# sai-soum/Diff-MST

Hardware: AMD Instinct MI355X
Metric: mixes/sec (8-track x 262144-sample fwd+bwd) (higher is better)
Workload: dtype f32

## Files before the change

### diff-mst_amd/csrc/mst_common.h

```cpp
#pragma once
#include <hip/hip_runtime.h>
#include <stdint.h>

#include "../../include/diffmst_hip.h"

namespace mst {

constexpr int kSections = 6;
constexpr int kStates = 2 * kSections;
#ifndef MST_COMP_WG
#define MST_COMP_WG 256
#endif
constexpr int kWG = MST_COMP_WG;
constexpr int kCompWaves = kWG / 64;
constexpr int kEqWG = 64;
constexpr int kEqChunk = 64;
constexpr int kCompChunk = 8;
constexpr int kScanThreads = 512;
constexpr int kScanLevels = 9;
constexpr int kPow = 1 + kScanLevels;
constexpr int kTile = kEqWG * kEqChunk;
constexpr int kPow1 = 12;
constexpr int kTri2 = 2 * 592;
constexpr int kFxDhChunks = 4;
constexpr int kWz = kEqChunk * 16;
constexpr int kMaxTiles1 = 64;

constexpr int RC_SOS = 0;
constexpr int RC_THR = 30;
constexpr int RC_KAPPA = 31;
constexpr int RC_KNEE = 32;
constexpr int RC_ALPHA = 33;
constexpr int RC_MAKEUP = 34;
constexpr int RC_ALPHA_C = 35;
constexpr int RC_PANL = 36;
constexpr int RC_PANR = 37;
constexpr int RC_GIN = 38;
constexpr int RC_LOG2A_C = 39;
constexpr int RC_SEND = 40;
constexpr int RC_AP = 44;
constexpr int RC_STRIDE = 64;

constexpr int CP_THR = 0, CP_KAPPA = 1, CP_KNEE = 2, CP_ALPHA = 3, CP_MAKEUP = 4, CP_PANL = 5, CP_PANR = 6, CP_SEND = 7;
constexpr int CP_COUNT = 8;
constexpr int EP_COUNT = 30;

constexpr float kDbPerLog2 = 6.02059991327962390f;
constexpr float kLog2PerDb = 0.16609640474436813f;
constexpr float kLn10Over20 = 0.11512925464970229f;
constexpr float kCompEps = 1e-8f;

__host__ __device__ inline int64_t round_up(int64_t a, int64_t b) { return (a + b - 1) / b * b; }
__host__ __device__ inline int filter_row(int sig, int split) { return sig < split ? sig : split + ((sig - split) >> 1); }

#if defined(__clang__)
using f2 = float __attribute__((ext_vector_type(2)));
__host__ __device__ __forceinline__ f2 f2_fma(f2 a, f2 b, f2 c) { return __builtin_elementwise_fma(a, b, c); }
#else
struct f2 {
    float x, y;
};
inline f2 operator*(f2 a, f2 b) { return f2{a.x * b.x, a.y * b.y}; }
inline f2 operator+(f2 a, f2 b) { return f2{a.x + b.x, a.y + b.y}; }
inline f2 f2_fma(f2 a, f2 b, f2 c) { return f2{fmaf(a.x, b.x, c.x), fmaf(a.y, b.y, c.y)}; }
#endif

template <typename T>
__device__ __forceinline__ T biquad_step(T x, const T* c, T& s1, T& s2) {
    T y = c[0] * x + s1;
    T n1 = c[1] * x + s2;
    s1 = n1 - c[3] * y;
    s2 = c[2] * x - c[4] * y;
    return y;
}
template <>
__device__ __forceinline__ float biquad_step<float>(float x, const float* c, float& s1, float& s2) {
    float y = fmaf(c[0], x, s1);
    float n1 = fmaf(c[1], x, s2);
    s1 = fmaf(-c[3], y, n1);
    s2 = fmaf(-c[4], y, c[2] * x);
    return y;
}

template <typename T>
__device__ __forceinline__ T cascade_step(T x, const T* c, T* st) {
#pragma unroll
    for (int k = 0; k < kSections; ++k) x = biquad_step<T>(x, c + 5 * k, st[2 * k], st[2 * k + 1]);
    return x;
}

template <typename T>
__device__ __forceinline__ T biquad_adj_step(T g, const T* c, T& r1, T& r2) {
    T p = g - c[3] * r1 - c[4] * r2;
    T xb = c[0] * p + c[1] * r1 + c[2] * r2;
    r2 = r1;
    r1 = p;
    return xb;
}
template <typename T>
__device__ __forceinline__ T cascade_adj_step(T g, const T* c, T* st) {
#pragma unroll
    for (int j = 0; j < kSections; ++j) {
        const int k = kSections - 1 - j;
        g = biquad_adj_step<T>(g, c + 5 * k, st[2 * j], st[2 * j + 1]);
    }
    return g;
}

__device__ __forceinline__ float4 load4(const float* __restrict__ row, int64_t i, int64_t n) {
    if (i + 3 < n && !((uintptr_t)(row + i) & 15)) return *reinterpret_cast<const float4*>(row + i);
    float4 v = make_float4(0.f, 0.f, 0.f, 0.f);
    if (i < n) v.x = row[i];
    if (i + 1 < n) v.y = row[i + 1];
    if (i + 2 < n) v.z = row[i + 2];
    if (i + 3 < n) v.w = row[i + 3];
    return v;
}
__device__ __forceinline__ void store4(float* __restrict__ row, int64_t i, int64_t n, float4 v) {
    if (i + 3 < n && !((uintptr_t)(row + i) & 15)) {
        *reinterpret_cast<float4*>(row + i) = v;
        return;
    }
    if (i < n) row[i] = v.x;
    if (i + 1 < n) row[i + 1] = v.y;
    if (i + 2 < n) row[i + 2] = v.z;
    if (i + 3 < n) row[i + 3] = v.w;
}
__device__ __forceinline__ float4 load4_shift(const float* __restrict__ row, int64_t i, int64_t n) {
    if (i >= 0 && i + 3 < n && !((uintptr_t)(row + i) & 15)) return *reinterpret_cast<const float4*>(row + i);
    float4 v = make_float4(0.f, 0.f, 0.f, 0.f);
    if (i >= 0 && i < n) v.x = row[i];
    if (i + 1 >= 0 && i + 1 < n) v.y = row[i + 1];
    if (i + 2 >= 0 && i + 2 < n) v.z = row[i + 2];
    if (i + 3 >= 0 && i + 3 < n) v.w = row[i + 3];
    return v;
}

__device__ __forceinline__ void wave_lds_sync() {
    __builtin_amdgcn_fence(__ATOMIC_RELEASE, "wavefront");
    __builtin_amdgcn_wave_barrier();
    __builtin_amdgcn_fence(__ATOMIC_ACQUIRE, "wavefront");
}

__device__ __forceinline__ void lds_barrier() {
    __builtin_amdgcn_fence(__ATOMIC_RELEASE, "workgroup", "local");
    __builtin_amdgcn_s_barrier();
    __builtin_amdgcn_fence(__ATOMIC_ACQUIRE, "workgroup", "local");
}
template <int LANES>
__device__ __forceinline__ void group_lds_sync() {
    if (LANES <= 64) wave_lds_sync();
    else lds_barrier();
}

template <int CTRL, int ROW_MASK>
__device__ __forceinline__ float dpp_add(float v) {
    return v + __int_as_float(__builtin_amdgcn_update_dpp(0, __float_as_int(v), CTRL, ROW_MASK, 0xf, true));
}
__device__ __forceinline__ float wave_sum(float v) {
    v = dpp_add<0x111, 0xf>(v);
    v = dpp_add<0x112, 0xf>(v);
    v = dpp_add<0x114, 0xf>(v);
    v = dpp_add<0x118, 0xf>(v);
    v = dpp_add<0x142, 0xa>(v);
    v = dpp_add<0x143, 0xc>(v);
    return __int_as_float(__builtin_amdgcn_readlane(__float_as_int(v), 63));
}

template <int CTRL, int ROW_MASK>
__device__ __forceinline__ double dpp_add_f64(double v) {
    const long long b = __double_as_longlong(v);
    const int lo = __builtin_amdgcn_update_dpp(0, (int)(b & 0xffffffffll), CTRL, ROW_MASK, 0xf, true);
    const int hi = __builtin_amdgcn_update_dpp(0, (int)(b >> 32), CTRL, ROW_MASK, 0xf, true);
    return v + __longlong_as_double(((long long)hi << 32) | (long long)(unsigned)lo);
}
__device__ __forceinline__ double wave_sum_f64(double v) {
    v = dpp_add_f64<0x111, 0xf>(v);
    v = dpp_add_f64<0x112, 0xf>(v);
    v = dpp_add_f64<0x114, 0xf>(v);
    v = dpp_add_f64<0x118, 0xf>(v);
    v = dpp_add_f64<0x142, 0xa>(v);
    v = dpp_add_f64<0x143, 0xc>(v);
    const long long b = __double_as_longlong(v);
    const int lo = __builtin_amdgcn_readlane((int)(b & 0xffffffffll), 63), hi = __builtin_amdgcn_readlane((int)(b >> 32), 63);
    return __longlong_as_double(((long long)hi << 32) | (long long)(unsigned)lo);
}

typedef unsigned long long gran_t;
#ifndef MST_GRAN_SPINS
#define MST_GRAN_SPINS (1 << 22)
#endif
constexpr int kStatusExchangeTimeout = 2000;
__device__ __forceinline__ void gran_give_up(int32_t* status) {
    if (status) atomicMax(status, kStatusExchangeTimeout);
}
__device__ __forceinline__ gran_t gran_load(const gran_t* g) { return __hip_atomic_load(g, __ATOMIC_RELAXED, __HIP_MEMORY_SCOPE_AGENT); }
__device__ __forceinline__ void gran_publish(gran_t* g, int64_t near_off, float v) {
#ifdef MST_GRAN_DROP_PUBLISH
    return;
#endif
    const gran_t x = ((gran_t)1 << 32) | (gran_t)(unsigned)__float_as_int(v);
    if (near_off) __hip_atomic_store(g + near_off, x, __ATOMIC_RELAXED, __HIP_MEMORY_SCOPE_WORKGROUP);
    __hip_atomic_store(g, x, __ATOMIC_RELAXED, __HIP_MEMORY_SCOPE_AGENT);
}
__device__ __forceinline__ float gran_wait(const gran_t* g, int64_t near_off, int32_t* status = nullptr) {
    const bool near = near_off;
    gran_t x = gran_load(near ? g + near_off : g);
    for (int spins = 0; (x >> 32) != 1; ++spins) {
        if (spins >= MST_GRAN_SPINS) {
            gran_give_up(status);
            return __int_as_float(0x7fc00000);
        }
        if (near && !(spins & 1)) x = gran_load(g);
        else {
            __builtin_amdgcn_s_sleep(1);
            x = gran_load(near ? g + near_off : g);
        }
    }
    return __int_as_float((int)(unsigned)x);
}
template <int NV>
__device__ __forceinline__ void gran_publish_vec(gran_t* g, int64_t near_off, const float* v, int src_lane, int lane) {
    float mine = 0.0f;
#pragma unroll
    for (int d = 0; d < NV; ++d) {
        const float t = __int_as_float(__builtin_amdgcn_readlane(__float_as_int(v[d]), src_lane));
        mine = lane == d ? t : mine;
    }
    if (lane < NV) gran_publish(g + lane, near_off, mine);
}
template <int NV>
__device__ __forceinline__ void gran_read_vec(const gran_t* g, int64_t near_off, float* out, bool active, int32_t* status) {
#pragma unroll
    for (int d = 0; d < NV; ++d) out[d] = 0.0f;
    if (!active) return;
    const bool has_near = near_off;
    bool use_near = has_near;
    gran_t x[NV];
    for (int spins = 0;; ++spins) {
        const gran_t* p = use_near ? g + near_off : g;
        bool ok = true;
#pragma unroll
        for (int d = 0; d < NV; ++d) x[d] = gran_load(p + d);
#pragma unroll
        for (int d = 0; d < NV; ++d) ok = ok && (x[d] >> 32) == 1;
        if (ok) break;
        if (spins >= MST_GRAN_SPINS) {
            gran_give_up(status);
#pragma unroll
            for (int d = 0; d < NV; ++d) x[d] = 0x7fc00000ull;
            break;
        }
        if (has_near) use_near = !use_near;
        if (!has_near || use_near) __builtin_amdgcn_s_sleep(1);
    }
#pragma unroll
    for (int d = 0; d < NV; ++d) out[d] = __int_as_float((int)(unsigned)x[d]);
}

__device__ __forceinline__ void row_block_xcd(int& row, int& step, int group = 1, int rows = 0, int skip_rows = 0) {
    const int nblk = gridDim.x;
    if (rows <= 0) rows = gridDim.y - skip_rows;
    if (group >= 1 && rows % (8 * group) == 0 && (nblk * skip_rows) % 8 == 0) {
        const int L = blockIdx.x + nblk * ((int)blockIdx.y - skip_rows), xcd = L & 7, k = L >> 3;
        const int per_group = group * nblk, gi = k / per_group, rem = k % per_group;
        row = (gi * 8 + xcd) * group + rem % group;
        step = rem / group;
    } else {
        row = blockIdx.y - skip_rows;
        step = blockIdx.x;
    }
}

struct Layout {
    int bs, T, R;
    int64_t N;
    int ncE, ncE_pad;
    int ncC, ncC_pad;
    int nblkE, nblkC;
    int nblkEt;
    int KE, KC;
    int ntE;
    int eq1;
    int apscan_fwd;
    int apscan_sh;
    int64_t rc_t, rc_m;
    int64_t powF_t, powF_m;
    int64_t powA_t, powA_m;
    int64_t powP_t, powP_m;
    int64_t u_t, gs_t, bus, v_m, gs_m;
    int64_t zE_t, sE_t, zE_m, sE_m;
    int64_t zS_t, sS_t, zS_m, sS_m;
    int64_t du_m, dbus, du_t;
    int64_t zQ_t, sQ_t, zQ_m, sQ_m;
    int64_t zA_t, sA_t, zA_m, sA_m;
    int64_t zP_t, sP_t, zP_m, sP_m;
    int64_t cp_t, cp_m, ep_t, ep_m;
    int64_t pow1F_t, pow1F_m, pow1A_t, pow1A_m;
    int64_t aggF_t, aggF_m, aggA_t, aggA_m;
    int64_t wzF_t, wzF_m, wzA_t, wzA_m;
    int64_t gran_f, gran_b;
    int64_t gran_nf, gran_nb;
    int64_t eqg_f, eqg_b;
    int64_t eqg_nf, eqg_nb;
    int fxS, fxTaps, fxK, fxBlk, fxBlkIr;
    int64_t fx_rc, fx_in, fx_wnf, fx_ir, fx_Xs, fx_Hs, fx_Ys, fx_dXs, fx_dHs, fx_dir, fx_din, fx_part, fx_Hf, fx_mix, fx_dry;
    int64_t total;
};

#ifndef MST_ROW_PAD
#define MST_ROW_PAD 0
#endif
inline int64_t row_stride(int64_t n) { return round_up(n, 4) + MST_ROW_PAD; }

inline Layout make_layout(const mst_console_desc* d) {
    Layout L{};
    L.bs = d->bs;
    L.T = d->n_tracks;
    L.R = d->bs * d->n_tracks;
    L.N = d->n_samples;
    L.ncE = (int)((L.N + kEqChunk - 1) / kEqChunk);
    L.ncE_pad = (int)round_up(L.ncE, 256);
    L.ncC = (int)((L.N + kCompChunk - 1) / kCompChunk);
    L.ncC_pad = (int)round_up(L.ncC, kWG);
    L.nblkE = L.ncE_pad / kEqWG;
    L.nblkC = L.ncC_pad / kWG;
    L.nblkEt = L.nblkC;
    L.KE = (L.ncE + kScanThreads - 1) / kScanThreads;
    if (L.KE > 8) L.KE = (int)round_up(L.KE, 8);
    L.KC = (L.ncC + kScanThreads - 1) / kScanThreads;
    L.ntE = (int)((L.N + kTile - 1) / kTile);
    L.eq1 = (L.ntE <= kMaxTiles1 && !(d->flags & MST_DEV_MULTIPASS_EQ)) ? 1 : 0;
    {
        int sh = 0;
        while ((L.KE << sh) < 64) ++sh;
        const bool pow2 = (L.KE << sh) == 64;
        L.apscan_fwd = (L.eq1 && pow2 && (d->flags & MST_USE_MASTER_BUS) && (d->flags & MST_SAVE_FOR_BACKWARD)) ? 1 : 0;
        L.apscan_sh = sh;
    }
    int64_t o = 0;
    auto take = [&](int64_t n) {
        int64_t at = o;
        o += round_up(n, 64);
        return at;
    };
    const int64_t R = L.R, B = L.bs, N = row_stride(L.N);
    L.rc_t = take((R + B) * RC_STRIDE);
    L.rc_m = L.rc_t + R * RC_STRIDE;
    L.powF_t = take((R + B) * kPow * 144);
    L.powF_m = L.powF_t + R * kPow * 144;
    L.powA_t = take((R + B) * kPow * 144);
    L.powA_m = L.powA_t + R * kPow * 144;
    L.powP_t = take((R + B) * 12 * kPow * 4);
    L.powP_m = L.powP_t + R * 12 * kPow * 4;
    L.u_t = take((R + 2 * B) * N);
    L.v_m = L.u_t + R * N;
    L.gs_t = take(R * N);
    L.bus = take(B * 2 * N);
    L.gs_m = take(B * N);
    L.zE_t = take(R * 12 * L.ncE_pad);
    L.sE_t = take(R * 12 * L.ncE_pad);
    L.zE_m = take(B * 2 * 12 * L.ncE_pad);
    L.sE_m = take(B * 2 * 12 * L.ncE_pad);
    L.zS_t = take(R * L.ncC_pad);
    L.sS_t = take(R * L.ncC_pad);
    L.zS_m = take(B * L.ncC_pad);
    L.sS_m = take(B * L.ncC_pad);
    L.du_t = take((R + 2 * B) * N);
    L.du_m = L.du_t + R * N;
    L.dbus = take(B * 2 * N);
    L.zQ_t = take(R * L.ncC_pad);
    L.sQ_t = take(R * L.ncC_pad);
    L.zQ_m = take(B * L.ncC_pad);
    L.sQ_m = take(B * L.ncC_pad);
    L.zA_t = take(R * 12 * L.ncE_pad);
    L.sA_t = take(R * 12 * L.ncE_pad);
    L.zA_m = take(B * 2 * 12 * L.ncE_pad);
    L.sA_m = take(B * 2 * 12 * L.ncE_pad);
    L.zP_t = take((R + 2 * B) * 24 * L.ncE_pad);
    L.zP_m = L.zP_t + R * 24 * L.ncE_pad;
    L.sP_t = take((R + 2 * B) * 24 * L.ncE_pad);
    L.sP_m = L.sP_t + R * 24 * L.ncE_pad;
    L.cp_t = take(R * L.nblkC * CP_COUNT);
    L.cp_m = take(B * L.nblkC * CP_COUNT);
    L.ep_t = take((R + 2 * B) * L.nblkEt * EP_COUNT);
    L.ep_m = L.ep_t + R * L.nblkEt * EP_COUNT;
    L.pow1F_t = take((R + B) * kTri2);
    L.pow1F_m = L.pow1F_t + R * kTri2;
    L.pow1A_t = take((R + B) * kTri2);
    L.pow1A_m = L.pow1A_t + R * kTri2;
    L.aggF_t = take((R + 2 * B) * kStates * kMaxTiles1);
    L.aggF_m = L.aggF_t + R * kStates * kMaxTiles1;
    L.aggA_t = take((R + 2 * B) * kStates * kMaxTiles1);
    L.aggA_m = L.aggA_t + R * kStates * kMaxTiles1;
    L.wzF_t = take((R + B) * kWz);
    L.wzF_m = L.wzF_t + R * kWz;
    L.wzA_t = take((R + B) * kWz);
    L.wzA_m = L.wzA_t + R * kWz;
    L.eqg_nf = (R + 2 * B) * kMaxTiles1 * kStates;
    L.eqg_nb = 2 * B * kMaxTiles1 * kStates;
    L.gran_nf = 2 * B * L.nblkC + 2 * L.eqg_nf;
    L.gran_nb = 2 * (R + B) * L.nblkC + 2 * L.eqg_nb;
    L.gran_f = take(2 * (L.gran_nf + L.gran_nb));
    L.gran_b = L.gran_f + 2 * L.gran_nf;
    L.eqg_f = L.gran_f + 2 * (2 * B * L.nblkC);
    L.eqg_b = L.gran_b + 2 * (2 * (R + B) * L.nblkC);
    if (d->flags & MST_USE_FX_BUS) {
        L.fxS = d->fx_ir_samples;
        L.fxTaps = d->fx_bandpass_taps;
        L.fxK = L.fxS / 4096;
        L.fxBlk = (int)((L.N + 4095) / 4096);
        L.fxBlkIr = (L.fxS + 1023) / 1024;
        L.fx_rc = take(B * 24);
        L.fx_in = take(B * 2 * N);
        L.fx_wnf = take(B * 2 * 12 * (int64_t)L.fxS);
        L.fx_ir = take(B * 2 * (int64_t)L.fxS);
        L.fx_Xs = take(B * (int64_t)L.fxBlk * 8192 * 2);
        L.fx_Hs = take(B * (int64_t)L.fxK * 8192 * 2);
        L.fx_Ys = take(B * (int64_t)L.fxBlk * 8192 * 2);
        L.fx_dXs = take(B * (int64_t)L.fxBlk * 8192 * 2);
        L.fx_dHs = take(B * (int64_t)L.fxK * 8192 * 2 * kFxDhChunks);
        L.fx_dir = take(B * 2 * (int64_t)L.fxS);
        L.fx_din = take(B * 2 * N);
        L.fx_part = take(B * (int64_t)L.fxBlkIr * 24);
        L.fx_Hf = take((int64_t)12 * 8192 * 2);
        L.fx_mix = take(B);
        L.fx_dry = take(B * (int64_t)L.fxBlk);
    }
    L.total = o;
    return L;
}

}
```

### diff-mst_amd/csrc/mst_console.hip

```cpp
#include "mst_kernels.h"
#include "mst_dev.h"

namespace mst {
static int check_desc(const mst_console_desc* d) {
    if (!d || d->bs <= 0 || d->n_tracks <= 0 || d->n_samples <= 0) return hipErrorInvalidValue;
    if (d->flags & MST_USE_FX_BUS) {
        if (d->fx_ir_samples < 4096 || d->fx_ir_samples % 4096 || d->fx_ir_samples > (1 << 20)) return hipErrorInvalidValue;
        if (d->fx_bandpass_taps < 1 || d->fx_bandpass_taps > 1023 || !(d->fx_bandpass_taps & 1)) return hipErrorInvalidValue;
    }
    if (!(d->flags & MST_USE_TRACK_PANNER)) return hipErrorInvalidValue;
    if (d->track_row_stride < d->n_samples) return hipErrorInvalidValue;
    if ((d->track_lookahead & 3) || (d->master_lookahead & 3) || d->track_lookahead < 0 || d->master_lookahead < 0)
        return hipErrorInvalidValue;
    return hipSuccess;
}
}

using namespace mst;

extern "C" int mst_abi_version(void) { return 11; }
MST_DEV_PROBE_STATE

extern "C" size_t mst_console_fx_tables_bytes(void) { return (size_t)8192 * 2 * sizeof(float); }
extern "C" int mst_console_fx_init_tables(void* tables, void* stream) {
    if (!tables) return hipErrorInvalidValue;
    launch_fx_tables((float*)tables, (hipStream_t)stream);
    return (int)hipGetLastError();
}

static FxPlan fx_plan(const Layout& L) {
    FxPlan p{};
    p.bs = L.bs;
    p.S = L.fxS;
    p.taps = L.fxTaps;
    p.K = L.fxK;
    p.nblk = L.fxBlk;
    p.nblk_ir = L.fxBlkIr;
    p.n = L.N;
    p.Ns = row_stride(L.N);
    p.rcfx = L.fx_rc; p.fx_in = L.fx_in; p.wnf = L.fx_wnf; p.ir = L.fx_ir; p.Xs = L.fx_Xs; p.Hs = L.fx_Hs; p.Ys = L.fx_Ys;
    p.dXs = L.fx_dXs; p.dHs = L.fx_dHs; p.dir = L.fx_dir; p.dfx_in = L.fx_din; p.fxpart = L.fx_part; p.Hf = L.fx_Hf; p.mixv = L.fx_mix; p.dry = L.fx_dry;
    return p;
}

static bool split_on(const mst_console_desc* d) {
    return (d->flags & MST_SPLIT_BATCH) && d->bs >= 2 && !(d->flags & MST_USE_FX_BUS) && !basic_path(d);
}
struct Halves {
    mst_console_desc da, db;
    int64_t ws_b;
    int64_t total;
};
static Halves make_halves(const mst_console_desc* d) {
    Halves h{*d, *d, 0, 0};
    h.da.bs = d->bs / 2;
    h.db.bs = d->bs - h.da.bs;
    h.da.flags &= ~MST_SPLIT_BATCH;
    h.db.flags &= ~MST_SPLIT_BATCH;
    h.ws_b = make_layout(&h.da).total;
    h.total = h.ws_b + make_layout(&h.db).total;
    return h;
}
static bool overlap_ok(const mst_console_overlap* ov) { return ov && ov->side_stream && ov->fork_event && ov->join_event; }

extern "C" size_t mst_console_workspace_bytes(const mst_console_desc* d) {
    if (check_desc(d) != hipSuccess) return 0;
    if (split_on(d)) return (size_t)make_halves(d).total * sizeof(float);
    return (size_t)make_layout(d).total * sizeof(float);
}

static int console_forward_impl(const mst_console_desc* d, const float* tracks, const float* track_params,
                                const float* fx_bus_params, const float* master_bus_params, const mst_console_fx* fx,
                                float* mix, float* mixed_tracks, int32_t* status, void* workspace, size_t workspace_bytes,
                                void* stream_, int32_t* status_host, void* status_event) {
    if (int e = check_desc(d)) return e;
    const Layout L = make_layout(d);
    if (!workspace || workspace_bytes < (size_t)L.total * sizeof(float) || ((uintptr_t)workspace & 255)) return hipErrorInvalidValue;
    if (!tracks || !track_params || !fx_bus_params || !master_bus_params || !mix || !status) return hipErrorInvalidValue;
    hipStream_t stream = (hipStream_t)stream_;
    float* ws = (float*)workspace;
    const int64_t n = L.N, Ns = row_stride(L.N);
    const bool save = d->flags & MST_SAVE_FOR_BACKWARD;
    const int aligned = (n % 4 == 0) && !((uintptr_t)mix & 15) && !((uintptr_t)mixed_tracks & 15);
    const bool t_comp = d->flags & MST_USE_TRACK_COMPRESSOR;
    const bool m_on = d->flags & MST_USE_MASTER_BUS;
    const bool o_on = d->flags & MST_USE_OUTPUT_FADER;
    const bool fx_on = d->flags & MST_USE_FX_BUS;
    if (fx_on && (!fx || !fx->noise || !fx->filters || !fx->tables)) return hipErrorInvalidValue;
    if (basic_path(d)) {
        BasicArgs ba{tracks, track_params, fx_bus_params, master_bus_params, mix, mixed_tracks, status, nullptr, nullptr, nullptr, nullptr, nullptr,
                     ws + L.cp_t, *d};
        launch_basic_forward(ba, stream);
        if (status_host) {
            (void)hipMemcpyAsync(status_host, status, sizeof(int32_t), hipMemcpyDeviceToHost, stream);
            if (status_event) (void)hipEventRecord((hipEvent_t)status_event, stream);
        }
        return (int)hipGetLastError();
    }

    PrepArgs pa{track_params, fx_bus_params, master_bus_params, ws + L.rc_t, ws + L.rc_m,
                ws + L.powF_t, ws + L.powF_m, ws + L.powA_t, ws + L.powA_m, ws + L.powP_t, ws + L.powP_m,
                ws + L.pow1F_t, ws + L.pow1F_m, ws + L.pow1A_t, ws + L.pow1A_m, ws + L.wzF_t, ws + L.wzF_m, ws + L.wzA_t, ws + L.wzA_m, fx_on ? ws + L.fx_rc : nullptr, fx_on ? ws + L.fx_mix : nullptr, status, L.R, L.bs, L.KE,
                L.eq1, *d, (gran_t*)(ws + L.gran_f), L.gran_nf + L.gran_nb, nullptr, 0, 0};
#ifndef MST_PREP_RIDER_MAX_BYTES
#define MST_PREP_RIDER_MAX_BYTES (128ll << 20)
#endif
    if (n % 4 == 0 && d->track_row_stride % 4 == 0 && !((uintptr_t)tracks & 15) && (int64_t)L.R * n * 4 <= MST_PREP_RIDER_MAX_BYTES) {
        pa.pf_src = tracks;
        pa.pf_stride = d->track_row_stride;
        pa.pf_n = n;
    }
    launch_prep(pa, stream);
    if (status_host && status) {
        (void)hipMemcpyAsync(status_host, status, sizeof(int32_t), hipMemcpyDeviceToHost, stream);
        if (status_event) (void)hipEventRecord((hipEvent_t)status_event, stream);
    }
    MST_DEV_PROBE_AT(0, stream);

    const float* p1F_t = L.eq1 ? ws + L.pow1F_t : nullptr;
    const float* p1F_m = L.eq1 ? ws + L.pow1F_m : nullptr;
    const float* sE_t = L.eq1 ? ws + L.zE_t : ws + L.sE_t;
    const float* sE_m = L.eq1 ? ws + L.zE_m : ws + L.sE_m;
    float* zP_t = save ? ws + L.zP_t : nullptr;
    float* zP_m = save ? ws + L.zP_m : nullptr;
    const bool zsin = L.eq1;
    const ZsIn zi_t{ws + L.wzF_t, (gran_t*)(ws + L.eqg_f), L.eqg_nf, status};
    const ZsIn zi_m{ws + L.wzF_m, (gran_t*)(ws + L.eqg_f) + (int64_t)L.R * kMaxTiles1 * kStates, L.eqg_nf, status};
#ifndef MST_ZSIN_MAX_TILES
#define MST_ZSIN_MAX_TILES 8192
#endif
    const bool zsin_t = zsin && t_comp && (int64_t)L.R * L.ntE <= MST_ZSIN_MAX_TILES;
    if (zsin_t) {}
    else if (L.eq1) launch_eq_zs_mfma(EQ_FWD, tracks, d->track_row_stride, ws + L.wzF_t, L.R, ws + L.zE_t, L.ncE_pad, n, L.R, stream, p1F_t, L.ntE, ws + L.aggF_t);
    else launch_cascade(EQ_FWD, false, tracks, d->track_row_stride, nullptr, 0, ws + L.rc_t, L.R, nullptr, ws + L.zE_t, L.ncE_pad, n, L.R, stream, p1F_t, L.ntE, ws + L.aggF_t);
    if (!L.eq1) launch_scan12(false, ws + L.zE_t, ws + L.sE_t, ws + L.powF_t, L.R, L.ncE, L.ncE_pad, L.KE, L.R, stream);
    if (t_comp)
        launch_cascade_run_gc(tracks, d->track_row_stride, ws + L.u_t, Ns, ws + L.rc_t, L.R, sE_t, L.ncE_pad, n, L.R,
                              ws + L.zS_t, L.nblkC, stream, p1F_t, L.ntE, ws + L.aggF_t, zP_t, zsin_t ? &zi_t : nullptr);
    else
        launch_cascade(EQ_FWD, true, tracks, d->track_row_stride, ws + L.u_t, Ns, ws + L.rc_t, L.R, sE_t, nullptr, L.ncE_pad, n, L.R, stream, p1F_t, L.ntE, ws + L.aggF_t, zP_t);
    const bool bus_is_mix = !m_on && !o_on;
    float* busp = bus_is_mix ? mix : ws + L.bus;
    const int64_t bus_stride = bus_is_mix ? n : Ns;
    TrackApplyArgs ta{ws + L.u_t, Ns, ws + L.rc_t, ws + L.zS_t, (save && t_comp) ? ws + L.gs_t : nullptr,
                      busp, bus_stride, mixed_tracks, fx_on ? ws + L.fx_in : nullptr,
                      L.T, L.ncC_pad, d->track_lookahead, t_comp ? 1 : 0, n, aligned};
    launch_apply_tracks(ta, L.bs, stream);
    MST_DEV_PROBE_AT(1, stream);
    if (fx_on) launch_fx_forward(fx_plan(L), fx->noise, fx->filters, (const float*)fx->tables, ws, busp, bus_stride, stream);

    if (m_on) {
        const bool apscan_m = L.apscan_fwd && zP_m && zP_t && p1F_m;
        const bool zsin_m = zsin && apscan_m;
        if (zsin_m) {}
        else if (L.eq1) launch_eq_zs_mfma(EQ_FWD, ws + L.bus, Ns, ws + L.wzF_m, 0, ws + L.zE_m, L.ncE_pad, n, 2 * L.bs, stream, p1F_m, L.ntE, ws + L.aggF_m);
        else launch_cascade(EQ_FWD, false, ws + L.bus, Ns, nullptr, 0, ws + L.rc_m, 0, nullptr, ws + L.zE_m, L.ncE_pad, n, 2 * L.bs, stream, p1F_m, L.ntE, ws + L.aggF_m);
        if (!L.eq1) launch_scan12(false, ws + L.zE_m, ws + L.sE_m, ws + L.powF_m, 0, L.ncE, L.ncE_pad, L.KE, 2 * L.bs, stream);
        if (apscan_m)
            launch_master_run_apscan(ws + L.bus, Ns, ws + L.v_m, Ns, ws + L.rc_m, sE_m, L.ncE_pad, n, 2 * L.bs, stream, p1F_m, L.ntE, ws + L.aggF_m, zP_m,
                                     ws + L.zP_t, ws + L.sP_t, ws + L.powP_t, L.R * 12, L.ncE, L.apscan_sh, EQ_FWD, zsin_m ? &zi_m : nullptr);
        else
            launch_cascade(EQ_FWD, true, ws + L.bus, Ns, ws + L.v_m, Ns, ws + L.rc_m, 0, sE_m, nullptr, L.ncE_pad, n, 2 * L.bs, stream, p1F_m, L.ntE, ws + L.aggF_m, zP_m);
        MasterApplyArgs ma{ws + L.v_m, Ns, ws + L.rc_m, ws + L.zS_m, save ? ws + L.gs_m : nullptr, mix, n,
                           L.ncC_pad, d->master_lookahead, 1, n, aligned, (gran_t*)(ws + L.gran_f), (int64_t)L.bs * L.nblkC, status};
        launch_apply_master(ma, L.bs, stream);
    } else if (o_on) {
        MasterApplyArgs ma{ws + L.bus, Ns, ws + L.rc_m, nullptr, nullptr, mix, n, L.ncC_pad, 0, 0, n, aligned};
        launch_apply_master(ma, L.bs, stream);
    }
    return (int)hipGetLastError();
}

extern "C" int mst_console_forward(const mst_console_desc* d, const float* tracks, const float* track_params,
                                   const float* fx_bus_params, const float* master_bus_params, const mst_console_fx* fx,
                                   float* mix, float* mixed_tracks, int32_t* status, void* workspace, size_t workspace_bytes,
                                   void* stream) {
    if (d && (d->flags & MST_SPLIT_BATCH)) return hipErrorInvalidValue;
    return console_forward_impl(d, tracks, track_params, fx_bus_params, master_bus_params, fx, mix, mixed_tracks, status, workspace,
                                workspace_bytes, stream, nullptr, nullptr);
}
extern "C" int mst_console_forward_overlapped(const mst_console_desc* d, const float* tracks, const float* track_params,
                                              const float* fx_bus_params, const float* master_bus_params, const mst_console_fx* fx,
                                              float* mix, float* mixed_tracks, int32_t* status, void* workspace, size_t workspace_bytes,
                                              void* stream, const mst_console_overlap* ov) {
    if (int e = check_desc(d)) return e;
    if (!split_on(d))
        return console_forward_impl(d, tracks, track_params, fx_bus_params, master_bus_params, fx, mix, mixed_tracks, status, workspace,
                                    workspace_bytes, stream, nullptr, nullptr);
    if (!overlap_ok(ov) || ov->side_stream == stream) return hipErrorInvalidValue;
    const Halves h = make_halves(d);
    if (!workspace || workspace_bytes < (size_t)h.total * sizeof(float) || ((uintptr_t)workspace & 255)) return hipErrorInvalidValue;
    if (!tracks || !track_params || !fx_bus_params || !master_bus_params || !mix || !status) return hipErrorInvalidValue;
    hipStream_t main_s = (hipStream_t)stream, side = (hipStream_t)ov->side_stream;
    const int64_t ba = h.da.bs, T = d->n_tracks, n = d->n_samples;
    if (int e = (int)hipEventRecord((hipEvent_t)ov->fork_event, main_s)) return e;
    if (int e = (int)hipStreamWaitEvent(side, (hipEvent_t)ov->fork_event, 0)) return e;
    float* ws = (float*)workspace;
    int e = console_forward_impl(&h.db, tracks + ba * T * d->track_row_stride, track_params + ba * T * MST_NUM_TRACK_PARAMS,
                                 fx_bus_params + ba * MST_NUM_FX_PARAMS, master_bus_params + ba * MST_NUM_MASTER_PARAMS, nullptr, mix + ba * 2 * n,
                                 mixed_tracks ? mixed_tracks + ba * 2 * T * n : nullptr, status, ws + h.ws_b,
                                 (size_t)(h.total - h.ws_b) * sizeof(float), side, nullptr, nullptr);
    if (!e)
        e = console_forward_impl(&h.da, tracks, track_params, fx_bus_params, master_bus_params, nullptr, mix, mixed_tracks, status, ws,
                                 (size_t)h.ws_b * sizeof(float), main_s, nullptr, nullptr);
    (void)hipEventRecord((hipEvent_t)ov->join_event, side);
    (void)hipStreamWaitEvent(main_s, (hipEvent_t)ov->join_event, 0);
    return e ? e : (int)hipGetLastError();
}
extern "C" int mst_console_forward_mirrored(const mst_console_desc* d, const float* tracks, const float* track_params,
                                            const float* fx_bus_params, const float* master_bus_params, const mst_console_fx* fx,
                                            float* mix, float* mixed_tracks, int32_t* status, void* workspace, size_t workspace_bytes,
                                            void* stream, int32_t* status_host, void* status_event) {
    if (!status || !status_host) return hipErrorInvalidValue;
    if (d && (d->flags & MST_SPLIT_BATCH)) return hipErrorInvalidValue;
    return console_forward_impl(d, tracks, track_params, fx_bus_params, master_bus_params, fx, mix, mixed_tracks, status, workspace,
                                workspace_bytes, stream, status_host, status_event);
}

static void allpole_scan(const Layout& L, float* ws, int nsig_all, hipStream_t stream) {
    if (!L.apscan_fwd) launch_scan2(ws + L.zP_t, ws + L.sP_t, ws + L.powP_t, L.R, L.ncE, L.ncE_pad, L.KE, nsig_all, stream);
}

extern "C" int mst_console_backward_prepare(const mst_console_desc* d, void* workspace, size_t workspace_bytes, void* stream_) {
    if (int e = check_desc(d)) return e;
    const Layout L = make_layout(d);
    if (!workspace || workspace_bytes < (size_t)L.total * sizeof(float) || ((uintptr_t)workspace & 255)) return hipErrorInvalidValue;
    if (!(d->flags & MST_SAVE_FOR_BACKWARD) || (d->flags & MST_SPLIT_BATCH)) return hipErrorInvalidValue;
    float* ws = (float*)workspace;
    const int nsig_all = L.R + ((d->flags & MST_USE_MASTER_BUS) ? 2 * L.bs : 0);
    allpole_scan(L, ws, nsig_all, (hipStream_t)stream_);
    return (int)hipGetLastError();
}

static int console_backward_impl(const mst_console_desc* d, const float* tracks, const float* track_params,
                                 const float* fx_bus_params, const float* master_bus_params, const mst_console_fx* fx,
                                 const float* grad_mix, const float* grad_mixed_tracks, float* grad_track_params,
                                 float* grad_fx_params, float* grad_master_params, float* grad_tracks, int32_t* status,
                                 void* workspace, size_t workspace_bytes, void* stream_) {
    if (int e = check_desc(d)) return e;
    const Layout L = make_layout(d);
    if (!workspace || workspace_bytes < (size_t)L.total * sizeof(float) || ((uintptr_t)workspace & 255)) return hipErrorInvalidValue;
    if (!(d->flags & MST_SAVE_FOR_BACKWARD)) return hipErrorInvalidValue;
    if (!track_params || !master_bus_params || !grad_mix || !grad_track_params || !grad_master_params) return hipErrorInvalidValue;
    hipStream_t stream = (hipStream_t)stream_;
    float* ws = (float*)workspace;
    const int64_t n = L.N, Ns = row_stride(L.N);
    const bool t_comp = d->flags & MST_USE_TRACK_COMPRESSOR;
    const bool m_on = d->flags & MST_USE_MASTER_BUS;
    const bool o_on = d->flags & MST_USE_OUTPUT_FADER;
    const bool fx_on = d->flags & MST_USE_FX_BUS;
    if (fx_on && (!fx || !fx->tables || !fx_bus_params)) return hipErrorInvalidValue;
    const int aligned = (n % 4 == 0) && !((uintptr_t)grad_mix & 15) && !((uintptr_t)grad_mixed_tracks & 15);
    if (basic_path(d)) {
        if (!tracks) return hipErrorInvalidValue;
        BasicArgs ba{tracks, track_params, fx_bus_params, master_bus_params, nullptr, nullptr, nullptr, grad_mix, grad_mixed_tracks,
                     grad_track_params, grad_master_params, grad_tracks, ws + L.cp_t, *d};
        launch_basic_backward(ba, stream);
        return (int)hipGetLastError();
    }

    const int nsig_all = L.R + (m_on ? 2 * L.bs : 0);
    if (!(d->flags & MST_BWD_PREPARED)) {
        allpole_scan(L, ws, nsig_all, stream);
    }

    const float* gbus = grad_mix;
    int64_t gbus_stride = n;
    if (m_on) {
        CompBwdArgs ca{ws + L.v_m, Ns, ws + L.gs_m, ws + L.rc_m, nullptr, ws + L.zQ_m, ws + L.du_m, ws + L.cp_m,
                       grad_mix, n, nullptr, nullptr, 0, 1, L.ncC_pad, d->master_lookahead, 1, n, aligned};
        ca.gran = (gran_t*)(ws + L.gran_b) + 2 * (int64_t)L.R * L.nblkC;
        ca.gran_near = (int64_t)L.bs * L.nblkC;
        ca.status = status;
        ca.s0 = ws + L.zQ_m;
        const bool master_cg_later = L.apscan_fwd;
        if (!master_cg_later) {
            ca.ap_s0 = ws + L.sP_m;
            ca.ap_nc_pad = L.ncE_pad;
            ca.ep = ws + L.ep_m;
        }
        launch_comp_bwd(true, ca, L.bs, stream);
        const float* p1A_m = L.eq1 ? ws + L.pow1A_m : nullptr;
        const bool zsin_a = L.eq1 && master_cg_later;
        const ZsIn zi_a{ws + L.wzA_m, (gran_t*)(ws + L.eqg_b), L.eqg_nb, status};
        if (zsin_a) {}
        else if (L.eq1) launch_eq_zs_mfma(EQ_ADJ, ws + L.du_m, Ns, ws + L.wzA_m, 0, ws + L.zA_m, L.ncE_pad, n, 2 * L.bs, stream, p1A_m, L.ntE, ws + L.aggA_m);
        else launch_cascade(EQ_ADJ, false, ws + L.du_m, Ns, nullptr, 0, ws + L.rc_m, 0, nullptr, ws + L.zA_m, L.ncE_pad, n, 2 * L.bs, stream, p1A_m, L.ntE, ws + L.aggA_m);
        if (!L.eq1) launch_scan12(true, ws + L.zA_m, ws + L.sA_m, ws + L.powA_m, 0, L.ncE, L.ncE_pad, L.KE, 2 * L.bs, stream);
        if (master_cg_later)
            launch_master_run_apscan(ws + L.du_m, Ns, ws + L.dbus, Ns, ws + L.rc_m, ws + L.zA_m, L.ncE_pad, n, 2 * L.bs, stream, p1A_m, L.ntE, ws + L.aggA_m,
                                     nullptr, ws + L.zP_m, ws + L.sP_m, ws + L.powP_m, 2 * L.bs * 12, L.ncE, L.apscan_sh, EQ_ADJ, zsin_a ? &zi_a : nullptr);
        else
            launch_cascade(EQ_ADJ, true, ws + L.du_m, Ns, ws + L.dbus, Ns, ws + L.rc_m, 0, L.eq1 ? ws + L.zA_m : ws + L.sA_m, nullptr, L.ncE_pad, n,
                           2 * L.bs, stream, p1A_m, L.ntE, ws + L.aggA_m);
        gbus = ws + L.dbus;
        gbus_stride = Ns;
    } else if (o_on) {
        CompBwdArgs ca{ws + L.bus, Ns, nullptr, ws + L.rc_m, nullptr, nullptr, ws + L.dbus, ws + L.cp_m,
                       grad_mix, n, nullptr, nullptr, 0, 1, L.ncC_pad, 0, 0, n, aligned};
        launch_comp_bwd(true, ca, L.bs, stream);
        gbus = ws + L.dbus;
        gbus_stride = Ns;
    } else {
        (void)hipMemsetAsync(ws + L.cp_m, 0, (size_t)L.bs * L.nblkC * CP_COUNT * sizeof(float), stream);
    }

    if (fx_on) launch_fx_backward(fx_plan(L), gbus, gbus_stride, (const float*)fx->tables, ws, stream);

    {
        CompBwdArgs ca{ws + L.u_t, Ns, ws + L.gs_t, ws + L.rc_t, nullptr, ws + L.zQ_t, ws + L.du_t, ws + L.cp_t,
                       gbus, gbus_stride, grad_mixed_tracks, fx_on ? ws + L.fx_din : nullptr, Ns, L.T, L.ncC_pad, d->track_lookahead,
                       t_comp ? 1 : 0, n, aligned};
        if (t_comp) {
            ca.gran = (gran_t*)(ws + L.gran_b);
            ca.gran_near = (int64_t)L.R * L.nblkC;
            ca.status = status;
            ca.s0 = ws + L.zQ_t;
        }
        ca.ap_s0 = ws + L.sP_t;
        ca.ap_nc_pad = L.ncE_pad;
        ca.ep = ws + L.ep_t;
        if (!grad_tracks) ca.du = nullptr;
        if (m_on && L.apscan_fwd) {
            ca.cg2_u = ws + L.v_m;
            ca.cg2_du = ws + L.du_m;
            ca.cg2_rc = ws + L.rc_m;
            ca.cg2_rows = 2 * L.bs;
        }
        launch_comp_bwd(false, ca, L.R, stream);
        if (grad_tracks) {
            const float* p1A_t = L.eq1 ? ws + L.pow1A_t : nullptr;
            if (L.eq1) launch_eq_zs_mfma(EQ_ADJ, ws + L.du_t, Ns, ws + L.wzA_t, L.R, ws + L.zA_t, L.ncE_pad, n, L.R, stream, p1A_t, L.ntE, ws + L.aggA_t);
            else launch_cascade(EQ_ADJ, false, ws + L.du_t, Ns, nullptr, 0, ws + L.rc_t, L.R, nullptr, ws + L.zA_t, L.ncE_pad, n, L.R, stream, p1A_t, L.ntE, ws + L.aggA_t);
            if (!L.eq1) launch_scan12(true, ws + L.zA_t, ws + L.sA_t, ws + L.powA_t, L.R, L.ncE, L.ncE_pad, L.KE, L.R, stream);
            launch_cascade(EQ_ADJ, true, ws + L.du_t, Ns, grad_tracks, n, ws + L.rc_t, L.R, L.eq1 ? ws + L.zA_t : ws + L.sA_t, nullptr, L.ncE_pad,
                           n, L.R, stream, p1A_t, L.ntE, ws + L.aggA_t);
        }
    }
    PrepBwdArgs pb{track_params, master_bus_params, ws + L.rc_t, ws + L.rc_m, ws + L.cp_t, ws + L.cp_m, ws + L.ep_t, ws + L.ep_m,
                   grad_track_params, grad_master_params, fx_bus_params, fx_on ? ws + L.fx_part : nullptr,
                   fx_on ? grad_fx_params : nullptr, L.fxBlkIr, fx_on ? ws + L.fx_mix : nullptr, fx_on ? ws + L.fx_dry : nullptr, L.fxBlk, L.R, L.bs, L.nblkC, L.nblkE, L.nblkEt, *d,
                   (gran_t*)(ws + L.gran_b), L.gran_nb};
    launch_prep_bwd(pb, stream);
    return (int)hipGetLastError();
}

extern "C" int mst_console_backward(const mst_console_desc* d, const float* tracks, const float* track_params,
                                    const float* fx_bus_params, const float* master_bus_params, const mst_console_fx* fx,
                                    const float* grad_mix, const float* grad_mixed_tracks, float* grad_track_params,
                                    float* grad_fx_params, float* grad_master_params, float* grad_tracks, int32_t* status,
                                    void* workspace, size_t workspace_bytes, void* stream) {
    if (d && (d->flags & MST_SPLIT_BATCH)) return hipErrorInvalidValue;
    return console_backward_impl(d, tracks, track_params, fx_bus_params, master_bus_params, fx, grad_mix, grad_mixed_tracks, grad_track_params,
                                 grad_fx_params, grad_master_params, grad_tracks, status, workspace, workspace_bytes, stream);
}
extern "C" int mst_console_backward_overlapped(const mst_console_desc* d, const float* tracks, const float* track_params,
                                               const float* fx_bus_params, const float* master_bus_params, const mst_console_fx* fx,
                                               const float* grad_mix, const float* grad_mixed_tracks, float* grad_track_params,
                                               float* grad_fx_params, float* grad_master_params, float* grad_tracks, int32_t* status,
                                               void* workspace, size_t workspace_bytes, void* stream, const mst_console_overlap* ov) {
    if (int e = check_desc(d)) return e;
    if (!split_on(d))
        return console_backward_impl(d, tracks, track_params, fx_bus_params, master_bus_params, fx, grad_mix, grad_mixed_tracks, grad_track_params,
                                     grad_fx_params, grad_master_params, grad_tracks, status, workspace, workspace_bytes, stream);
    if (!overlap_ok(ov) || ov->side_stream == stream || (d->flags & MST_BWD_PREPARED)) return hipErrorInvalidValue;
    const Halves h = make_halves(d);
    if (!workspace || workspace_bytes < (size_t)h.total * sizeof(float) || ((uintptr_t)workspace & 255)) return hipErrorInvalidValue;
    if (!track_params || !master_bus_params || !grad_mix || !grad_track_params || !grad_master_params) return hipErrorInvalidValue;
    hipStream_t main_s = (hipStream_t)stream, side = (hipStream_t)ov->side_stream;
    const int64_t ba = h.da.bs, T = d->n_tracks, n = d->n_samples;
    if (int e = (int)hipEventRecord((hipEvent_t)ov->fork_event, main_s)) return e;
    if (int e = (int)hipStreamWaitEvent(side, (hipEvent_t)ov->fork_event, 0)) return e;
    float* ws = (float*)workspace;
    int e = console_backward_impl(&h.db, tracks ? tracks + ba * T * d->track_row_stride : nullptr, track_params + ba * T * MST_NUM_TRACK_PARAMS,
                                  fx_bus_params ? fx_bus_params + ba * MST_NUM_FX_PARAMS : nullptr, master_bus_params + ba * MST_NUM_MASTER_PARAMS, nullptr,
                                  grad_mix + ba * 2 * n, grad_mixed_tracks ? grad_mixed_tracks + ba * 2 * T * n : nullptr,
                                  grad_track_params + ba * T * MST_NUM_TRACK_PARAMS, nullptr, grad_master_params + ba * MST_NUM_MASTER_PARAMS,
                                  grad_tracks ? grad_tracks + ba * T * n : nullptr, status, ws + h.ws_b, (size_t)(h.total - h.ws_b) * sizeof(float), side);
    if (!e)
        e = console_backward_impl(&h.da, tracks, track_params, fx_bus_params, master_bus_params, nullptr, grad_mix, grad_mixed_tracks, grad_track_params,
                                  nullptr, grad_master_params, grad_tracks, status, ws, (size_t)h.ws_b * sizeof(float), main_s);
    (void)hipEventRecord((hipEvent_t)ov->join_event, side);
    (void)hipStreamWaitEvent(main_s, (hipEvent_t)ov->join_event, 0);
    return e ? e : (int)hipGetLastError();
}
```

### diff-mst_amd/csrc/mst_eq.hip

```cpp
#include "mst_kernels.h"
#include "mst_mat.h"
#include "mst_compdev.h"

namespace mst {

#ifndef MST_EQ_SLAB
#define MST_EQ_SLAB 16
#endif
constexpr int kSlab = MST_EQ_SLAB;
constexpr int kLdw = kSlab + 4;
constexpr int kNSlab = kEqChunk / kSlab;
constexpr int kSlabVec = kSlab / 4;
constexpr int kFetch = kEqWG * kSlabVec / kEqWG;

struct SlabRegs {
    float4 v[kFetch];
};
template <bool FAST>
__device__ __forceinline__ void slab_fetch(SlabRegs& r, const float* __restrict__ row, int64_t tile_base, int j, int64_t n, int tid) {
#pragma unroll
    for (int q0 = 0; q0 < kFetch; ++q0) {
        const int q = tid + kEqWG * q0;
        const int lane = q / kSlabVec;
        const int i = (q % kSlabVec) * 4;
        const int64_t at = tile_base + (int64_t)lane * kEqChunk + j * kSlab + i;
        r.v[q0] = FAST ? *reinterpret_cast<const float4*>(row + at) : load4(row, at, n);
    }
}
__device__ __forceinline__ void slab_stash(const SlabRegs& r, float* __restrict__ tile, int tid) {
#pragma unroll
    for (int q0 = 0; q0 < kFetch; ++q0) {
        const int q = tid + kEqWG * q0;
        *reinterpret_cast<float4*>(&tile[(q / kSlabVec) * kLdw + (q % kSlabVec) * 4]) = r.v[q0];
    }
}
template <bool FAST>
__device__ __forceinline__ void slab_store(const float* __restrict__ tile, float* __restrict__ row, int64_t tile_base,
                                           int j, int64_t n, int tid) {
#pragma unroll
    for (int q0 = 0; q0 < kFetch; ++q0) {
        const int q = tid + kEqWG * q0;
        const int lane = q / kSlabVec;
        const int i = (q % kSlabVec) * 4;
        const int64_t at = tile_base + (int64_t)lane * kEqChunk + j * kSlab + i;
        const float4 v = *reinterpret_cast<const float4*>(&tile[lane * kLdw + i]);
        if (FAST) *reinterpret_cast<float4*>(row + at) = v;
        else store4(row, at, n, v);
    }
}

__device__ __forceinline__ bool tile_fast(const float* row, int64_t tile_base, int64_t n) {
    return tile_base + kTile <= n && !((uintptr_t)row & 15);
}

typedef float f32x4_t __attribute__((vector_size(16)));
template <bool FAST>
__device__ __forceinline__ void zs_inline(const float* __restrict__ row, int64_t tile_base, int64_t n, const float* __restrict__ w,
                                          float* __restrict__ tile, float* st, int lane) {
    constexpr int kPitch = kStates + 1;
    const int li = lane & 15, g = lane >> 4;
    float4 x[4][4];
#pragma unroll
    for (int m = 0; m < 4; ++m)
#pragma unroll
        for (int s = 0; s < 4; ++s) {
            const int64_t at = tile_base + (int64_t)(16 * m + li) * kEqChunk + 16 * s + 4 * g;
            x[m][s] = FAST ? *reinterpret_cast<const float4*>(row + at) : load4(row, at, n);
        }
    float wb[16];
#pragma unroll
    for (int s = 0; s < 4; ++s)
#pragma unroll
        for (int e = 0; e < 4; ++e) wb[4 * s + e] = w[(16 * s + 4 * g + e) * 16 + li];
    f32x4_t acc[4];
#pragma unroll
    for (int m = 0; m < 4; ++m) {
        acc[m] = f32x4_t{0.f, 0.f, 0.f, 0.f};
#pragma unroll
        for (int s = 0; s < 4; ++s) {
            const float xs[4] = {x[m][s].x, x[m][s].y, x[m][s].z, x[m][s].w};
#pragma unroll
            for (int e = 0; e < 4; ++e) acc[m] = __builtin_amdgcn_mfma_f32_16x16x4f32(xs[e], wb[4 * s + e], acc[m], 0, 0, 0);
        }
    }
    if (li < kStates) {
#pragma unroll
        for (int m = 0; m < 4; ++m)
#pragma unroll
            for (int r = 0; r < 4; ++r) tile[(16 * m + 4 * g + r) * kPitch + li] = acc[m][r];
    }
    wave_lds_sync();
#pragma unroll
    for (int dd = 0; dd < kStates; ++dd) st[dd] = tile[lane * kPitch + dd];
    wave_lds_sync();
}

template <int DIR, bool MODE_RUN, bool FUSE_GC, bool SCAN1, bool FAST, bool FUSE_AP, bool ZSIN = false>
__device__ __forceinline__ void cascade_body(const float* __restrict__ in, int64_t in_stride,
                                                 float* __restrict__ out, int64_t out_stride,
                                                 const float* __restrict__ rc, int split,
                                                 const float* __restrict__ s0, float* __restrict__ z,
                                                 int nc_pad, int64_t n, float* __restrict__ zs_comp,
                                                 int nblk_comp, const float* __restrict__ pw1, int ntiles,
                                                 float* __restrict__ agg, float* __restrict__ tile, float* __restrict__ zp,
                                                 const int sig, const int bx, const ZsIn zi = ZsIn{}) {
    static_assert(!ZSIN || (MODE_RUN && SCAN1), "the in-launch zero-state pass belongs to the SCAN1 run");
    const int tid = threadIdx.x;
    const int64_t tile_base = (int64_t)bx * kEqWG * kEqChunk;
    const int chunk = bx * kEqWG + tid;
    const float* inrow = in + (int64_t)sig * in_stride;
    float* outrow = MODE_RUN ? out + (int64_t)sig * out_stride : nullptr;
    auto order = [](int jj) { return (DIR == EQ_FWD) ? jj : kNSlab - 1 - jj; };
    const int pos = DIR == EQ_FWD ? tid : kEqWG - 1 - tid;
    const float* tab = SCAN1 ? pw1 + (int64_t)filter_row(sig, split) * kTri2 : nullptr;
    TabRegs tlo, thi;
    if (SCAN1) tab_fetch(tlo, tab, tid);
    float st[kStates];
    const int wt = DIR == EQ_FWD ? bx : ntiles - 1 - bx;
    if (ZSIN) {
        zs_inline<FAST>(inrow, tile_base, n, zi.wz + (int64_t)filter_row(sig, split) * kWz, tile, st, tid);
        gran_t* gq = zi.gran + ((int64_t)sig * kMaxTiles1) * kStates;
        {
            float sc[kStates];
#pragma unroll
            for (int i = 0; i < kStates; ++i) sc[i] = st[i];
            tab_stash(tlo, tile, tid);
            wave_lds_sync();
            wave_scan_tri<DIR == EQ_ADJ>(sc, tile, pos);
            wave_lds_sync();
            gran_publish_vec<kStates>(gq + (int64_t)wt * kStates, zi.gran_near, sc, DIR == EQ_FWD ? kEqWG - 1 : 0, tid);
        }
#pragma unroll
        for (int i = 0; i < kStates; ++i) st[i] = dpp_get<(DIR == EQ_ADJ) ? 0x130 : 0x138>(st[i]);
    }
    SlabRegs pre;
    slab_fetch<FAST>(pre, inrow, tile_base, order(0), n, tid);

    const float* coef = rc + (int64_t)filter_row(sig, split) * RC_STRIDE + RC_SOS;
    float c[5 * kSections];
#pragma unroll
    for (int i = 0; i < 5 * kSections; ++i) c[i] = coef[i];
    if (MODE_RUN && SCAN1) {
        tab_fetch(thi, tab + kTriFloats, tid);
        const int nb = DIR == EQ_FWD ? chunk - 1 : chunk + 1;
        if (!ZSIN) {
#pragma unroll
            for (int i = 0; i < kStates; ++i) st[i] = pos > 0 ? s0[((int64_t)sig * kStates + i) * nc_pad + nb] : 0.0f;
        }
        if (wt > 0) {
            float zz[kStates];
            if (ZSIN) {
                gran_read_vec<kStates>(zi.gran + ((int64_t)sig * kMaxTiles1 + tid) * kStates, zi.gran_near, zz, tid < wt, zi.status);
            } else {
#pragma unroll
                for (int d = 0; d < kStates; ++d) zz[d] = tid < wt ? agg[((int64_t)sig * kStates + d) * kMaxTiles1 + tid] : 0.0f;
            }
            tab_stash(thi, tile, tid);
            wave_lds_sync();
            wave_scan_tri<false>(zz, tile, tid);
#pragma unroll
            for (int d = 0; d < kStates; ++d) {
                const float S = __shfl(zz[d], wt - 1);
                if (pos == 0) st[d] = S;
            }
            wave_lds_sync();
        }
        tab_stash(tlo, tile, tid);
        wave_lds_sync();
        wave_scan_tri<DIR == EQ_ADJ>(st, tile, pos);
        wave_lds_sync();
    } else {
#pragma unroll
        for (int i = 0; i < kStates; ++i)
            st[i] = MODE_RUN ? s0[((int64_t)sig * kStates + i) * nc_pad + chunk] : 0.0f;
    }
    float* mine = &tile[tid * kLdw];
    CompK ck{};
    float zacc = 0.0f;
    if (FUSE_GC) ck = load_comp(rc + (int64_t)filter_row(sig, split) * RC_STRIDE);
    f2 nk1[kSections], nk2[kSections], w1[kSections], w2[kSections];
    if (FUSE_AP) {
#pragma unroll
        for (int s = 0; s < kSections; ++s) {
            nk1[s] = f2{-c[5 * s + 3], -coef[RC_AP - RC_SOS + 3 * s]};
            nk2[s] = f2{-c[5 * s + 4], -coef[RC_AP - RC_SOS + 3 * s + 1]};
            w1[s] = w2[s] = f2{0.0f, 0.0f};
        }
    }

#ifndef MST_EQ_PACKED
#define MST_EQ_PACKED 0
#endif
    f2 sp[kSections], cb[kSections], can[kSections];
    if (DIR == EQ_FWD && MST_EQ_PACKED) {
#pragma unroll
        for (int s = 0; s < kSections; ++s) {
            sp[s] = f2{st[2 * s], st[2 * s + 1]};
            cb[s] = f2{c[5 * s + 1], c[5 * s + 2]};
            can[s] = f2{-c[5 * s + 3], -c[5 * s + 4]};
        }
    }
    auto step_fwd = [&](float x) {
        if (!MST_EQ_PACKED) return cascade_step<float>(x, c, st);
#pragma unroll
        for (int s = 0; s < kSections; ++s) {
            const float y = fmaf(c[5 * s], x, sp[s].x);
            sp[s] = f2_fma(can[s], f2{y, y}, f2_fma(cb[s], f2{x, x}, f2{sp[s].y, 0.0f}));
            x = y;
        }
        return x;
    };
    for (int jj = 0; jj < kNSlab; ++jj) {
        const int j = order(jj);
        slab_stash(pre, tile, tid);
        wave_lds_sync();
        if (jj + 1 < kNSlab) slab_fetch<FAST>(pre, inrow, tile_base, order(jj + 1), n, tid);
        if (DIR == EQ_FWD) {
#pragma unroll
            for (int i4 = 0; i4 < kSlab; i4 += 4) {
                float4 v = *reinterpret_cast<float4*>(&mine[i4]);
                v.x = step_fwd(v.x);
                v.y = step_fwd(v.y);
                v.z = step_fwd(v.z);
                v.w = step_fwd(v.w);
                if (MODE_RUN) *reinterpret_cast<float4*>(&mine[i4]) = v;
                if (FUSE_AP) {
                    const float ys[4] = {v.x, v.y, v.z, v.w};
#pragma unroll
                    for (int t = 0; t < 4; ++t) {
#pragma unroll
                        for (int s = 0; s < kSections; ++s) {
                            const f2 wn = f2_fma(nk2[s], w2[s], f2_fma(nk1[s], w1[s], f2{ys[t], ys[t]}));
                            w2[s] = w1[s];
                            w1[s] = wn;
                        }
                    }
                }
                if (FUSE_GC) {
                    float dd;
                    zacc = fmaf(ck.alpha, zacc, ck.oma * gain_computer(v.x, ck, dd));
                    zacc = fmaf(ck.alpha, zacc, ck.oma * gain_computer(v.y, ck, dd));
                    zacc = fmaf(ck.alpha, zacc, ck.oma * gain_computer(v.z, ck, dd));
                    zacc = fmaf(ck.alpha, zacc, ck.oma * gain_computer(v.w, ck, dd));
                }
            }
        } else {
#pragma unroll
            for (int i4 = kSlab - 4; i4 >= 0; i4 -= 4) {
                float4 v = *reinterpret_cast<float4*>(&mine[i4]);
                v.w = cascade_adj_step<float>(v.w, c, st);
                v.z = cascade_adj_step<float>(v.z, c, st);
                v.y = cascade_adj_step<float>(v.y, c, st);
                v.x = cascade_adj_step<float>(v.x, c, st);
                if (MODE_RUN) *reinterpret_cast<float4*>(&mine[i4]) = v;
            }
        }
        wave_lds_sync();
        if (MODE_RUN) {
            slab_store<FAST>(tile, outrow, tile_base, j, n, tid);
            wave_lds_sync();
        }
    }
    if (DIR == EQ_FWD && MST_EQ_PACKED) {
#pragma unroll
        for (int s = 0; s < kSections; ++s) {
            st[2 * s] = sp[s].x;
            st[2 * s + 1] = sp[s].y;
        }
    }
    if (!MODE_RUN) {
#pragma unroll
        for (int i = 0; i < kStates; ++i) z[((int64_t)sig * kStates + i) * nc_pad + chunk] = st[i];
        if (SCAN1) {
            tab_stash(tlo, tile, tid);
            wave_lds_sync();
            wave_scan_tri<DIR == EQ_ADJ>(st, tile, pos);
            if (pos == kEqWG - 1) {
#pragma unroll
                for (int i = 0; i < kStates; ++i) agg[((int64_t)sig * kStates + i) * kMaxTiles1 + wt] = st[i];
            }
        }
    }
    if (FUSE_AP) {
#pragma unroll
        for (int s = 0; s < kSections; ++s) {
            const int64_t base = ((int64_t)sig * 24 + 4 * s) * nc_pad + chunk;
            zp[base] = w1[s].x;
            zp[base + nc_pad] = w2[s].x;
            zp[base + 2 * (int64_t)nc_pad] = w1[s].y;
            zp[base + 3 * (int64_t)nc_pad] = w2[s].y;
        }
    }
    if (FUSE_GC) {
        constexpr int kBlkLanes = kWG * kCompChunk / kEqChunk;
        const float l2a64 = 8.0f * rc[(int64_t)filter_row(sig, split) * RC_STRIDE + RC_LOG2A_C];
        float p = __builtin_amdgcn_exp2f(l2a64);
        const int lseg = tid & (kBlkLanes - 1);
#pragma unroll
        for (int d = 1; d < kBlkLanes; d <<= 1) {
            const float o = __shfl_up(zacc, d);
            if (lseg >= d) zacc = fmaf(p, o, zacc);
            p *= p;
        }
        const int blk = chunk / kBlkLanes;
        if (lseg == kBlkLanes - 1 && blk < nblk_comp) zs_comp[(int64_t)sig * nblk_comp + blk] = zacc;
    }
}

template <int DIR, bool MODE_RUN, bool FUSE_GC = false, bool SCAN1 = false, bool FUSE_AP = false>
#ifndef MST_EQ_RUN_W
#define MST_EQ_RUN_W 4
#endif
__global__ __launch_bounds__(kEqWG, (MODE_RUN && FUSE_GC && FUSE_AP) ? MST_EQ_RUN_W : 1) void k_cascade(const float* __restrict__ in, int64_t in_stride,
                                                 float* __restrict__ out, int64_t out_stride,
                                                 const float* __restrict__ rc, int split,
                                                 const float* __restrict__ s0, float* __restrict__ z,
                                                 int nc_pad, int64_t n, float* __restrict__ zs_comp = nullptr,
                                                 int nblk_comp = 0, const float* __restrict__ pw1 = nullptr, int ntiles = 0,
                                                 float* __restrict__ agg = nullptr, float* __restrict__ zp = nullptr) {
    static_assert(!FUSE_AP || (MODE_RUN && DIR == EQ_FWD), "the all-pole bank rides on the forward run only");
    __shared__ __attribute__((aligned(16))) float tile[kEqWG * kLdw > kTriFloats ? kEqWG * kLdw : kTriFloats];
    const int64_t tile_base = (int64_t)blockIdx.x * kTile;
    const bool fast = tile_fast(in + (int64_t)blockIdx.y * in_stride, tile_base, n) &&
                      (!MODE_RUN || !((uintptr_t)(out + (int64_t)blockIdx.y * out_stride) & 15));
    if (fast) cascade_body<DIR, MODE_RUN, FUSE_GC, SCAN1, true, FUSE_AP>(in, in_stride, out, out_stride, rc, split, s0, z, nc_pad, n, zs_comp, nblk_comp, pw1, ntiles, agg, tile, zp, blockIdx.y, blockIdx.x);
    else cascade_body<DIR, MODE_RUN, FUSE_GC, SCAN1, false, FUSE_AP>(in, in_stride, out, out_stride, rc, split, s0, z, nc_pad, n, zs_comp, nblk_comp, pw1, ntiles, agg, tile, zp, blockIdx.y, blockIdx.x);
}

template <int DIR, bool FUSE_GC, bool FUSE_AP>
__global__ __launch_bounds__(kEqWG, (FUSE_GC && FUSE_AP) ? MST_EQ_RUN_W : 1) void k_cascade_zsin(const float* __restrict__ in, int64_t in_stride,
                                                 float* __restrict__ out, int64_t out_stride,
                                                 const float* __restrict__ rc, int split, int nc_pad, int64_t n,
                                                 float* __restrict__ zs_comp, int nblk_comp, const float* __restrict__ pw1, int ntiles,
                                                 float* __restrict__ zp, ZsIn zi) {
    __shared__ __attribute__((aligned(16))) float tile[kEqWG * kLdw > kTriFloats ? kEqWG * kLdw : kTriFloats];
    int sig, step;
    row_block_xcd(sig, step);
    const int bx = DIR == EQ_FWD ? step : ntiles - 1 - step;
    const int64_t tile_base = (int64_t)bx * kTile;
    const bool fast = tile_fast(in + (int64_t)sig * in_stride, tile_base, n) && !((uintptr_t)(out + (int64_t)sig * out_stride) & 15);
    if (fast) cascade_body<DIR, true, FUSE_GC, true, true, FUSE_AP, true>(in, in_stride, out, out_stride, rc, split, nullptr, nullptr, nc_pad, n, zs_comp, nblk_comp, pw1, ntiles, nullptr, tile, zp, sig, bx, zi);
    else cascade_body<DIR, true, FUSE_GC, true, false, FUSE_AP, true>(in, in_stride, out, out_stride, rc, split, nullptr, nullptr, nc_pad, n, zs_comp, nblk_comp, pw1, ntiles, nullptr, tile, zp, sig, bx, zi);
}

template <int DIR>
__global__ __launch_bounds__(kEqWG) void k_eq_zs_mfma(const float* __restrict__ in, int64_t in_stride, const float* __restrict__ wz, int split,
                                                     float* __restrict__ z, int nc_pad, int64_t n, const float* __restrict__ pw1, int ntiles,
                                                     float* __restrict__ agg) {
    constexpr int kPitch = kStates + 1;
    __shared__ __attribute__((aligned(16))) float tile[kEqWG * kPitch > kTriFloats ? kEqWG * kPitch : kTriFloats];
    const int lane = threadIdx.x, sig = blockIdx.y;
    const int64_t tile_base = (int64_t)blockIdx.x * kTile;
    const float* row = in + (int64_t)sig * in_stride;
    const int frow = filter_row(sig, split);
    TabRegs tlo;
    tab_fetch(tlo, pw1 + (int64_t)frow * kTri2, lane);
    float st[kStates];
    if (tile_fast(row, tile_base, n)) zs_inline<true>(row, tile_base, n, wz + (int64_t)frow * kWz, tile, st, lane);
    else zs_inline<false>(row, tile_base, n, wz + (int64_t)frow * kWz, tile, st, lane);
    const int chunk0 = blockIdx.x * kEqWG;
#pragma unroll
    for (int dd = 0; dd < kStates; ++dd) z[((int64_t)sig * kStates + dd) * nc_pad + chunk0 + lane] = st[dd];
    tab_stash(tlo, tile, lane);
    wave_lds_sync();
    const int pos = DIR == EQ_FWD ? lane : kEqWG - 1 - lane;
    wave_scan_tri<DIR == EQ_ADJ>(st, tile, pos);
    if (pos == kEqWG - 1) {
        const int wt = DIR == EQ_FWD ? (int)blockIdx.x : ntiles - 1 - (int)blockIdx.x;
#pragma unroll
        for (int dd = 0; dd < kStates; ++dd) agg[((int64_t)sig * kStates + dd) * kMaxTiles1 + wt] = st[dd];
    }
}
void launch_eq_zs_mfma(int dir, const float* in, int64_t in_stride, const float* wz, int split, float* z, int nc_pad, int64_t n, int nsig,
                       hipStream_t stream, const float* pw1, int ntiles, float* agg) {
    const dim3 grid(ntiles, nsig), block(kEqWG);
    if (dir == EQ_FWD) hipLaunchKernelGGL(HIP_KERNEL_NAME(k_eq_zs_mfma<EQ_FWD>), grid, block, 0, stream, in, in_stride, wz, split, z, nc_pad, n, pw1, ntiles, agg);
    else hipLaunchKernelGGL(HIP_KERNEL_NAME(k_eq_zs_mfma<EQ_ADJ>), grid, block, 0, stream, in, in_stride, wz, split, z, nc_pad, n, pw1, ntiles, agg);
}

template <bool FAST>
__device__ __forceinline__ void allpole_scan_tile(const float* __restrict__ z0, float* __restrict__ o0, const float* __restrict__ tab, int nc,
                                                  int nc_pad, int sh, float* __restrict__ tileA, float* __restrict__ tileB, int tid) {
    const float* z1 = z0 + nc_pad;
    float* o1 = o0 + nc_pad;
    SlabRegs ra[kNSlab], rb[kNSlab];
#pragma unroll
    for (int j = 0; j < kNSlab; ++j) {
        slab_fetch<FAST>(ra[j], z0, 0, j, nc, tid);
        slab_fetch<FAST>(rb[j], z1, 0, j, nc, tid);
    }
    const float p00 = tab[0], p01 = tab[1], p10 = tab[2], p11 = tab[3];
    float a = 0.0f, b = 0.0f;
    float* mineA = &tileA[tid * kLdw];
    float* mineB = &tileB[tid * kLdw];
#pragma unroll
    for (int j = 0; j < kNSlab; ++j) {
        slab_stash(ra[j], tileA, tid);
        slab_stash(rb[j], tileB, tid);
        wave_lds_sync();
#pragma unroll
        for (int i4 = 0; i4 < kSlab; i4 += 4) {
            const float4 va = *reinterpret_cast<const float4*>(&mineA[i4]), vb = *reinterpret_cast<const float4*>(&mineB[i4]);
            const float xa[4] = {va.x, va.y, va.z, va.w}, xb[4] = {vb.x, vb.y, vb.z, vb.w};
#pragma unroll
            for (int t = 0; t < 4; ++t) {
                const float na = fmaf(p01, b, fmaf(p00, a, xa[t])), nb = fmaf(p11, b, fmaf(p10, a, xb[t]));
                a = na;
                b = nb;
            }
        }
        wave_lds_sync();
    }
    const int lanes = (nc + kEqChunk - 1) / kEqChunk;
    for (int j = 0; (1 << j) < lanes; ++j) {
        const float* T = tab + (1 + sh + j) * 4;
        const float oa = __shfl_up(a, 1 << j), ob = __shfl_up(b, 1 << j);
        if (tid >= (1 << j)) {
            a = fmaf(T[1], ob, fmaf(T[0], oa, a));
            b = fmaf(T[3], ob, fmaf(T[2], oa, b));
        }
    }
    float ea = __shfl_up(a, 1), eb = __shfl_up(b, 1);
    if (tid == 0) ea = eb = 0.0f;
#pragma unroll
    for (int j = 0; j < kNSlab; ++j) {
        slab_stash(ra[j], tileA, tid);
        slab_stash(rb[j], tileB, tid);
        wave_lds_sync();
#pragma unroll
        for (int i4 = 0; i4 < kSlab; i4 += 4) {
            const float4 va = *reinterpret_cast<const float4*>(&mineA[i4]), vb = *reinterpret_cast<const float4*>(&mineB[i4]);
            const float xa[4] = {va.x, va.y, va.z, va.w}, xb[4] = {vb.x, vb.y, vb.z, vb.w};
            float ya[4], yb[4];
#pragma unroll
            for (int t = 0; t < 4; ++t) {
                ya[t] = ea;
                yb[t] = eb;
                const float na = fmaf(p01, eb, fmaf(p00, ea, xa[t])), nb = fmaf(p11, eb, fmaf(p10, ea, xb[t]));
                ea = na;
                eb = nb;
            }
            *reinterpret_cast<float4*>(&mineA[i4]) = make_float4(ya[0], ya[1], ya[2], ya[3]);
            *reinterpret_cast<float4*>(&mineB[i4]) = make_float4(yb[0], yb[1], yb[2], yb[3]);
        }
        wave_lds_sync();
        slab_store<FAST>(tileA, o0, 0, j, nc, tid);
        slab_store<FAST>(tileB, o1, 0, j, nc, tid);
        wave_lds_sync();
    }
}

struct ApScanArgs {
    const float* z;
    float* s0;
    const float* tab;
    int jobs, nc, nc_pad, sh;
    int stereo;
};
template <int DIR, bool ZSIN>
__global__ __launch_bounds__(kEqWG) void k_master_run_apscan(const float* __restrict__ in, int64_t in_stride, float* __restrict__ out,
                                                           int64_t out_stride, const float* __restrict__ rc, const float* __restrict__ s0,
                                                           int nc_pad, int64_t n, const float* __restrict__ pw1, int ntiles,
                                                           float* __restrict__ agg, float* __restrict__ zp, int nsig, ApScanArgs sc, ZsIn zi) {
    __shared__ __attribute__((aligned(16))) float tile[2 * kEqWG * kLdw > kTriFloats ? 2 * kEqWG * kLdw : kTriFloats];
    if ((int)blockIdx.y >= nsig) {
        const int job = ((int)blockIdx.y - nsig) * gridDim.x + blockIdx.x;
        if (job >= sc.jobs) return;
        const float* z0 = sc.z + (int64_t)job * 2 * sc.nc_pad;
        float* o0 = sc.s0 + (int64_t)job * 2 * sc.nc_pad;
        const int trow = sc.stereo ? ((job / 12) >> 1) * 12 + job % 12 : job;
        const float* tab = sc.tab + (int64_t)trow * kPow * 4;
        if (sc.nc == kTile) allpole_scan_tile<true>(z0, o0, tab, sc.nc, sc.nc_pad, sc.sh, tile, tile + kEqWG * kLdw, threadIdx.x);
        else allpole_scan_tile<false>(z0, o0, tab, sc.nc, sc.nc_pad, sc.sh, tile, tile + kEqWG * kLdw, threadIdx.x);
        return;
    }
    int sig = blockIdx.y, bx = blockIdx.x;
    if (ZSIN) {
        int step;
        row_block_xcd(sig, step, 1, nsig);
        bx = DIR == EQ_FWD ? step : ntiles - 1 - step;
    }
    const int64_t tile_base = (int64_t)bx * kTile;
    const bool fast = tile_fast(in + (int64_t)sig * in_stride, tile_base, n) && !((uintptr_t)(out + (int64_t)sig * out_stride) & 15);
    constexpr bool AP = DIR == EQ_FWD;
    if (fast) cascade_body<DIR, true, false, true, true, AP, ZSIN>(in, in_stride, out, out_stride, rc, 0, s0, nullptr, nc_pad, n, nullptr, 0, pw1, ntiles, agg, tile, zp, sig, bx, zi);
    else cascade_body<DIR, true, false, true, false, AP, ZSIN>(in, in_stride, out, out_stride, rc, 0, s0, nullptr, nc_pad, n, nullptr, 0, pw1, ntiles, agg, tile, zp, sig, bx, zi);
}
void launch_master_run_apscan(const float* in, int64_t in_stride, float* out, int64_t out_stride, const float* rc, const float* s0, int nc_pad,
                              int64_t n, int nsig, hipStream_t stream, const float* pw1, int ntiles, float* agg, float* zp,
                              const float* sc_z, float* sc_s0, const float* sc_tab, int sc_jobs, int sc_nc, int sc_sh, int dir, const ZsIn* zi) {
    const ApScanArgs sc{sc_z, sc_s0, sc_tab, sc_jobs, sc_nc, nc_pad, sc_sh, dir == EQ_ADJ ? 1 : 0};
    const dim3 grid(ntiles, nsig + (sc_jobs + ntiles - 1) / ntiles), block(kEqWG);
    const ZsIn z0 = zi ? *zi : ZsIn{};
#define MST_LAUNCH_MRA(D, Z) \
    hipLaunchKernelGGL(HIP_KERNEL_NAME(k_master_run_apscan<D, Z>), grid, block, 0, stream, in, in_stride, out, out_stride, rc, s0, nc_pad, n, pw1, ntiles, agg, zp, nsig, sc, z0)
    if (dir == EQ_FWD) {
        if (z0.wz) MST_LAUNCH_MRA(EQ_FWD, true);
        else MST_LAUNCH_MRA(EQ_FWD, false);
    } else {
        if (z0.wz) MST_LAUNCH_MRA(EQ_ADJ, true);
        else MST_LAUNCH_MRA(EQ_ADJ, false);
    }
#undef MST_LAUNCH_MRA
}

void launch_cascade(int dir, bool run, const float* in, int64_t in_stride, float* out, int64_t out_stride, const float* rc,
                    int split, const float* s0, float* z, int nc_pad, int64_t n, int nsig, hipStream_t stream, const float* pw1,
                    int ntiles, float* agg, float* zp) {
    const dim3 grid(pw1 ? ntiles : nc_pad / kEqWG, nsig), block(kEqWG);
    float* const nozs = nullptr;
    if (zp && dir == EQ_FWD && run) {
        if (pw1)
            hipLaunchKernelGGL(HIP_KERNEL_NAME(k_cascade<EQ_FWD, true, false, true, true>), grid, block, 0, stream, in, in_stride, out,
                               out_stride, rc, split, s0, z, nc_pad, n, nozs, 0, pw1, ntiles, agg, zp);
        else
            hipLaunchKernelGGL(HIP_KERNEL_NAME(k_cascade<EQ_FWD, true, false, false, true>), grid, block, 0, stream, in, in_stride, out,
                               out_stride, rc, split, s0, z, nc_pad, n, nozs, 0, pw1, ntiles, agg, zp);
        return;
    }
#define MST_LAUNCH_CASCADE(D, R, S) \
    hipLaunchKernelGGL(HIP_KERNEL_NAME(k_cascade<D, R, false, S>), grid, block, 0, stream, in, in_stride, out, out_stride, rc, \
                       split, s0, z, nc_pad, n, nozs, 0, pw1, ntiles, agg, nozs)
    if (pw1) {
        if (dir == EQ_FWD && !run) MST_LAUNCH_CASCADE(EQ_FWD, false, true);
        else if (dir == EQ_FWD) MST_LAUNCH_CASCADE(EQ_FWD, true, true);
        else if (!run) MST_LAUNCH_CASCADE(EQ_ADJ, false, true);
        else MST_LAUNCH_CASCADE(EQ_ADJ, true, true);
    } else {
        if (dir == EQ_FWD && !run) MST_LAUNCH_CASCADE(EQ_FWD, false, false);
        else if (dir == EQ_FWD) MST_LAUNCH_CASCADE(EQ_FWD, true, false);
        else if (!run) MST_LAUNCH_CASCADE(EQ_ADJ, false, false);
        else MST_LAUNCH_CASCADE(EQ_ADJ, true, false);
    }
#undef MST_LAUNCH_CASCADE
}

void launch_cascade_run_gc(const float* in, int64_t in_stride, float* out, int64_t out_stride, const float* rc, int split,
                           const float* s0, int nc_pad, int64_t n, int nsig, float* zs_comp, int nblk_comp, hipStream_t stream,
                           const float* pw1, int ntiles, float* agg, float* zp, const ZsIn* zi) {
    static_assert(kWG * kCompChunk % kEqChunk == 0 && kEqWG % (kWG * kCompChunk / kEqChunk) == 0, "a compressor block must be a power-of-two group of EQ lanes");
    const dim3 grid(pw1 ? ntiles : nc_pad / kEqWG, nsig), block(kEqWG);
    if (zi && zi->wz && pw1) {
        if (zp) hipLaunchKernelGGL(HIP_KERNEL_NAME(k_cascade_zsin<EQ_FWD, true, true>), grid, block, 0, stream, in, in_stride, out, out_stride, rc, split, nc_pad, n, zs_comp, nblk_comp, pw1, ntiles, zp, *zi);
        else hipLaunchKernelGGL(HIP_KERNEL_NAME(k_cascade_zsin<EQ_FWD, true, false>), grid, block, 0, stream, in, in_stride, out, out_stride, rc, split, nc_pad, n, zs_comp, nblk_comp, pw1, ntiles, zp, *zi);
        return;
    }
    if (zp) {
        if (pw1)
            hipLaunchKernelGGL(HIP_KERNEL_NAME(k_cascade<EQ_FWD, true, true, true, true>), grid, block, 0, stream, in, in_stride, out, out_stride,
                               rc, split, s0, (float*)nullptr, nc_pad, n, zs_comp, nblk_comp, pw1, ntiles, agg, zp);
        else
            hipLaunchKernelGGL(HIP_KERNEL_NAME(k_cascade<EQ_FWD, true, true, false, true>), grid, block, 0, stream, in, in_stride, out, out_stride,
                               rc, split, s0, (float*)nullptr, nc_pad, n, zs_comp, nblk_comp, pw1, ntiles, agg, zp);
        return;
    }
    if (pw1)
        hipLaunchKernelGGL(HIP_KERNEL_NAME(k_cascade<EQ_FWD, true, true, true>), grid, block, 0, stream, in, in_stride, out, out_stride,
                           rc, split, s0, (float*)nullptr, nc_pad, n, zs_comp, nblk_comp, pw1, ntiles, agg, (float*)nullptr);
    else
        hipLaunchKernelGGL(HIP_KERNEL_NAME(k_cascade<EQ_FWD, true, true, false>), grid, block, 0, stream, in, in_stride, out, out_stride,
                           rc, split, s0, (float*)nullptr, nc_pad, n, zs_comp, nblk_comp, pw1, ntiles, agg, (float*)nullptr);
}

}
```

### diff-mst_amd/csrc/mst_kernels.h

```cpp
#pragma once
#include "mst_common.h"

namespace mst {

enum { EQ_FWD = 0, EQ_ADJ = 1 };

struct PrepArgs {
    const float* track_params;
    const float* fx_params;
    const float* master_params;
    float* rc_t;
    float* rc_m;
    float* powF_t; float* powF_m;
    float* powA_t; float* powA_m;
    float* powP_t; float* powP_m;
    float* pow1F_t; float* pow1F_m;
    float* pow1A_t; float* pow1A_m;
    float* wzF_t; float* wzF_m;
    float* wzA_t; float* wzA_m;
    float* rc_fx;
    float* fx_mix;
    int32_t* status;
    int R, bs;
    int KE;
    int eq1;
    mst_console_desc d;
    gran_t* gran;
    int64_t gran_n;
    const float* pf_src;
    int64_t pf_stride, pf_n;
};
struct PrepBwdArgs {
    const float* track_params;
    const float* master_params;
    const float* rc_t;
    const float* rc_m;
    const float* cp_t; const float* cp_m;
    const float* ep_t; const float* ep_m;
    float* grad_track_params;
    float* grad_master_params;
    const float* fx_params;
    const float* fx_part;
    float* grad_fx_params;
    int nblkF;
    const float* fx_mix;
    const float* fx_dry;
    int nblkX;
    int R, bs, nblkC, nblkE;
    int nblkEt;
    mst_console_desc d;
    gran_t* gran;
    int64_t gran_n;
};
constexpr int kBasicMaxTracks = 256;
struct BasicArgs {
    const float* tracks;
    const float* track_params;
    const float* fx_params;
    const float* master_params;
    float* mix;
    float* mixed;
    int32_t* status;
    const float* grad_mix;
    const float* grad_mixed;
    float* grad_track_params;
    float* grad_master_params;
    float* grad_tracks;
    float* part;
    mst_console_desc d;
};
inline bool basic_path(const mst_console_desc* d) {
    const uint32_t stages = MST_USE_TRACK_EQ | MST_USE_TRACK_COMPRESSOR | MST_USE_FX_BUS | MST_USE_MASTER_BUS | MST_USE_OUTPUT_FADER;
    return !(d->flags & stages) && (d->flags & MST_USE_TRACK_PANNER) && d->n_tracks <= kBasicMaxTracks && !(d->flags & MST_DEV_MULTIPASS_EQ);
}
void launch_basic_forward(const BasicArgs& a, hipStream_t stream);
void launch_basic_backward(const BasicArgs& a, hipStream_t stream);
void launch_prep(const PrepArgs& a, hipStream_t stream);
void launch_prep_bwd(const PrepBwdArgs& a, hipStream_t stream);

struct ZsIn {
    const float* wz;
    gran_t* gran;
    int64_t gran_near;
    int32_t* status;
};
void launch_cascade(int dir, bool run, const float* in, int64_t in_stride, float* out, int64_t out_stride, const float* rc,
                    int split, const float* s0, float* z, int nc_pad, int64_t n, int nsig, hipStream_t stream,
                    const float* pw1 = nullptr, int ntiles = 0, float* agg = nullptr, float* zp = nullptr);
void launch_cascade_run_gc(const float* in, int64_t in_stride, float* out, int64_t out_stride, const float* rc, int split,
                           const float* s0, int nc_pad, int64_t n, int nsig, float* zs_comp, int nblk_comp, hipStream_t stream,
                           const float* pw1 = nullptr, int ntiles = 0, float* agg = nullptr, float* zp = nullptr, const ZsIn* zi = nullptr);
void launch_eq_zs_mfma(int dir, const float* in, int64_t in_stride, const float* wz, int split, float* z, int nc_pad, int64_t n, int nsig,
                       hipStream_t stream, const float* pw1, int ntiles, float* agg);
void launch_master_run_apscan(const float* in, int64_t in_stride, float* out, int64_t out_stride, const float* rc, const float* s0, int nc_pad,
                              int64_t n, int nsig, hipStream_t stream, const float* pw1, int ntiles, float* agg, float* zp,
                              const float* sc_z, float* sc_s0, const float* sc_tab, int sc_jobs, int sc_nc, int sc_sh, int dir = EQ_FWD,
                              const ZsIn* zi = nullptr);

void launch_scan12(bool reverse, const float* z, float* s0, const float* tab, int split, int nc, int nc_pad, int K, int nsig,
                   hipStream_t stream);
void launch_scan2(const float* z, float* s0, const float* tab, int split, int nc, int nc_pad, int K, int nsig, hipStream_t stream);

struct TrackApplyArgs {
    const float* u;
    int64_t stride;
    const float* rc;
    const float* s0;
    float* gs;
    float* bus;
    int64_t bus_stride;
    float* mixed;
    float* fx;
    int T, nc_pad, lookahead, comp_on;
    int64_t n;
    int aligned;
};
struct MasterApplyArgs {
    const float* v;
    int64_t stride;
    const float* rc;
    const float* s0;
    float* gs;
    float* out;
    int64_t out_stride;
    int nc_pad, lookahead, comp_on;
    int64_t n;
    int aligned;
    gran_t* gran;
    int64_t gran_near;
    int32_t* status;
};
struct CompBwdArgs {
    const float* u;
    int64_t stride;
    const float* gs;
    const float* rc;
    const float* s0;
    float* zq;
    float* du;
    float* part;
    const float* gup;
    int64_t gup_stride;
    const float* gmixed;
    const float* gfx;
    int64_t gfx_stride;
    int T, nc_pad, lookahead, comp_on;
    int64_t n;
    int aligned;
    const float* ap_s0;
    int ap_nc_pad;
    float* ep;
    const float* cg2_u;
    const float* cg2_du;
    const float* cg2_rc;
    int cg2_rows;
    gran_t* gran;
    int64_t gran_near;
    int32_t* status;
};
void launch_apply_tracks(const TrackApplyArgs& a, int bs, hipStream_t stream);
void launch_apply_master(const MasterApplyArgs& a, int bs, hipStream_t stream);
void launch_comp_bwd(bool master, const CompBwdArgs& a, int rows, hipStream_t stream);

struct FxPlan {
    int bs, S, taps, K, nblk, nblk_ir;
    int64_t n, Ns;
    int64_t rcfx, fx_in, wnf, ir, Xs, Hs, Ys, dXs, dHs, dir, dfx_in, fxpart, Hf, mixv, dry;
};
void launch_fx_forward(const FxPlan& p, const float* noise, const float* filters, const float* tables, float* ws, float* bus,
                       int64_t bus_stride, hipStream_t stream);
void launch_fx_backward(const FxPlan& p, const float* dbus, int64_t dbus_stride, const float* tables, float* ws, hipStream_t stream);
void launch_fx_tables(float* tables, hipStream_t stream);

}
```

### diff-mst_amd/csrc/mst_params.hip

```cpp
#include "mst_kernels.h"

namespace mst {

__device__ void design_section_f32(int kind, float gain_db, float freq, float q, float sr, float* out) {
#pragma clang fp contract(off)
    const float A = (float)exp2((double)(gain_db / 40.0f) * 3.321928094887362);
    const float w0 = 6.283185307179586f * (freq / sr);
    double sn64, cw64;
    sincos((double)w0, &sn64, &cw64);
    const float sn = (float)sn64;
    const float cw = (float)cw64;
    const float alpha = sn / (2.0f * q);
    const float sA = sqrtf(A);
    float b0, b1, b2, a0, a1, a2;
    if (kind == 1) {
        const float aA = alpha * A;
        const float aoA = alpha / A;
        b0 = 1.0f + aA;
        b1 = -2.0f * cw;
        b2 = 1.0f - aA;
        a0 = 1.0f + aoA;
        a1 = -2.0f * cw;
        a2 = 1.0f - aoA;
    } else {
        const float Ap1 = A + 1.0f, Am1 = A - 1.0f;
        const float t = (2.0f * sA) * alpha;
        const float m1 = Am1 * cw, p1 = Ap1 * cw;
        if (kind == 0) {
            b0 = A * ((Ap1 - m1) + t);
            b1 = (2.0f * A) * (Am1 - p1);
            b2 = A * ((Ap1 - m1) - t);
            a0 = (Ap1 + m1) + t;
            a1 = -2.0f * (Am1 + p1);
            a2 = (Ap1 + m1) - t;
        } else {
            b0 = A * ((Ap1 + m1) + t);
            b1 = (-2.0f * A) * (Am1 + p1);
            b2 = A * ((Ap1 + m1) - t);
            a0 = (Ap1 - m1) + t;
            a1 = 2.0f * (Am1 - p1);
            a2 = (Ap1 - m1) - t;
        }
    }
    out[0] = b0 / a0;
    out[1] = b1 / a0;
    out[2] = b2 / a0;
    out[3] = a1 / a0;
    out[4] = a2 / a0;
}

struct D3 {
    double v, d[3];
};
__device__ inline D3 dconst(double c) { return D3{c, {0, 0, 0}}; }
__device__ inline D3 operator+(D3 a, D3 b) { return D3{a.v + b.v, {a.d[0] + b.d[0], a.d[1] + b.d[1], a.d[2] + b.d[2]}}; }
__device__ inline D3 operator-(D3 a, D3 b) { return D3{a.v - b.v, {a.d[0] - b.d[0], a.d[1] - b.d[1], a.d[2] - b.d[2]}}; }
__device__ inline D3 operator*(D3 a, D3 b) {
    return D3{a.v * b.v, {a.d[0] * b.v + a.v * b.d[0], a.d[1] * b.v + a.v * b.d[1], a.d[2] * b.v + a.v * b.d[2]}};
}
__device__ inline D3 operator/(D3 a, D3 b) {
    const double r = 1.0 / b.v, q = a.v * r;
    return D3{q, {(a.d[0] - q * b.d[0]) * r, (a.d[1] - q * b.d[1]) * r, (a.d[2] - q * b.d[2]) * r}};
}
__device__ inline D3 dscale(D3 a, double s) { return D3{a.v * s, {a.d[0] * s, a.d[1] * s, a.d[2] * s}}; }
__device__ inline D3 dfun(D3 a, double f, double fp) { return D3{f, {a.d[0] * fp, a.d[1] * fp, a.d[2] * fp}}; }

__device__ void design_section_dual(int kind, double gain_db, double freq, double q, double sr, D3* out) {
    D3 g{gain_db, {1, 0, 0}}, f{freq, {0, 1, 0}}, qq{q, {0, 0, 1}};
    const double Av = exp2(gain_db / 40.0 * 3.321928094887362);
    D3 A = dfun(g, Av, Av * 2.302585092994046 / 40.0);
    D3 w0 = dscale(f, 6.283185307179586 / sr);
    double snv, csv;
    sincos(w0.v, &snv, &csv);
    D3 sn = dfun(w0, snv, csv);
    D3 cw = dfun(w0, csv, -snv);
    D3 alpha = sn / dscale(qq, 2.0);
    const double sAv = sqrt(Av);
    D3 sA = dfun(A, sAv, 0.5 / sAv);
    D3 one = dconst(1.0);
    D3 b0, b1, b2, a0, a1, a2;
    if (kind == 1) {
        b0 = one + alpha * A;
        b1 = dscale(cw, -2.0);
        b2 = one - alpha * A;
        a0 = one + alpha / A;
        a1 = dscale(cw, -2.0);
        a2 = one - alpha / A;
    } else {
        D3 Ap1 = A + one, Am1 = A - one, t = dscale(sA * alpha, 2.0);
        if (kind == 0) {
            b0 = A * (Ap1 - Am1 * cw + t);
            b1 = dscale(A * (Am1 - Ap1 * cw), 2.0);
            b2 = A * (Ap1 - Am1 * cw - t);
            a0 = Ap1 + Am1 * cw + t;
            a1 = dscale(Am1 + Ap1 * cw, -2.0);
            a2 = Ap1 + Am1 * cw - t;
        } else {
            b0 = A * (Ap1 + Am1 * cw + t);
            b1 = dscale(A * (Am1 + Ap1 * cw), -2.0);
            b2 = A * (Ap1 + Am1 * cw - t);
            a0 = Ap1 - Am1 * cw + t;
            a1 = dscale(Am1 - Ap1 * cw, 2.0);
            a2 = Ap1 - Am1 * cw - t;
        }
    }
    out[0] = b0 / a0;
    out[1] = b1 / a0;
    out[2] = b2 / a0;
    out[3] = a1 / a0;
    out[4] = a2 / a0;
}

__device__ __forceinline__ float denorm(float v, float lo, float hi) {
#pragma clang fp contract(off)
    return v * (hi - lo) + lo;
}
__device__ __forceinline__ int section_kind(int k) { return k == 0 ? 0 : (k == 5 ? 2 : 1); }

__device__ __forceinline__ void mat12_mul(const double* A, const double* B, double* C, int e) {
    const int i = e / 12, j = e % 12;
    double acc = 0.0;
#pragma unroll
    for (int k = 0; k < 12; ++k) acc = fma(A[i * 12 + k], B[k * 12 + j], acc);
    C[e] = acc;
}

__global__ __launch_bounds__(320) void k_prep(PrepArgs a) {
    __shared__ double mats[2][3][144];
    __shared__ double wv[2][kEqChunk][12];
    __shared__ double dblk[2][2][kSections][4];
    __shared__ float coef[32];
    const int row = blockIdx.x, tid = threadIdx.x;
    if (blockIdx.y >= 2) {
        if (row < a.R && a.pf_src) {
            const float4* src = reinterpret_cast<const float4*>(a.pf_src + (int64_t)row * a.pf_stride);
            const int nseg = gridDim.y - 2, seg = blockIdx.y - 2;
            const int64_t nv = a.pf_n >> 2, per = (nv + nseg - 1) / nseg, v0 = seg * per, v1 = v0 + per < nv ? v0 + per : nv;
            for (int64_t g0 = v0 + tid; g0 < v1; g0 += 320 * 8) {
                float4 v[8];
#pragma unroll
                for (int u = 0; u < 8; ++u) v[u] = g0 + 320 * u < v1 ? src[g0 + 320 * u] : make_float4(0.f, 0.f, 0.f, 0.f);
#if defined(__clang__)
#pragma unroll
                for (int u = 0; u < 8; ++u) asm volatile("" ::"v"(v[u].x), "v"(v[u].y), "v"(v[u].z), "v"(v[u].w));
#endif
            }
        }
        return;
    }
    for (int64_t i = ((int64_t)blockIdx.y * gridDim.x + blockIdx.x) * 320 + tid; i < a.gran_n; i += (int64_t)gridDim.x * 2 * 320) a.gran[i] = 0ull;
    const bool is_master = row >= a.R;
    const int mrow = row - a.R;
    const mst_console_desc& d = a.d;
    const float sr = d.sample_rate;
    const float* p = is_master ? a.master_params + (int64_t)mrow * MST_NUM_MASTER_PARAMS
                               : a.track_params + (int64_t)row * MST_NUM_TRACK_PARAMS;
    const float* lo = is_master ? d.master_lo : d.track_lo;
    const float* hi = is_master ? d.master_hi : d.track_hi;
    float* rc = is_master ? a.rc_m + (int64_t)mrow * RC_STRIDE : a.rc_t + (int64_t)row * RC_STRIDE;
    const int eq0 = is_master ? 0 : 1;
    const int cmp0 = is_master ? 18 : 19;
    const int np = is_master ? MST_NUM_MASTER_PARAMS : MST_NUM_TRACK_PARAMS;

    const bool check = !(d.flags & MST_NO_RANGE_CHECK);
    if (check && tid < np) {
        const float v = p[tid];
        if (v < 0.0f || v > 1.0f) atomicMax(a.status, 1000 - (1 + (is_master ? 52 : 0) + tid));
    }
    if (check && is_master && tid >= 32 && tid < 32 + 24) {
        const float v = a.fx_params[(int64_t)mrow * MST_NUM_FX_PARAMS + (tid - 32)];
        if (v < 0.0f || v > 1.0f) atomicMax(a.status, 1000 - (1 + 27 + (tid - 32)));
    }

    const bool eq_on = is_master ? (d.flags & MST_USE_MASTER_BUS) : (d.flags & MST_USE_TRACK_EQ);
    const bool comp_on = is_master ? (d.flags & MST_USE_MASTER_BUS) : (d.flags & MST_USE_TRACK_COMPRESSOR);
    const bool gin_on = is_master ? (d.flags & MST_USE_MASTER_BUS) : (d.flags & MST_USE_TRACK_INPUT_FADER);

    if (tid < kSections) {
        float c[5] = {1.f, 0.f, 0.f, 0.f, 0.f};
        if (eq_on) {
            const int i = eq0 + 3 * tid;
            design_section_f32(section_kind(tid), denorm(p[i], lo[i], hi[i]), denorm(p[i + 1], lo[i + 1], hi[i + 1]),
                               denorm(p[i + 2], lo[i + 2], hi[i + 2]), sr, c);
        }
        for (int j = 0; j < 5; ++j) coef[5 * tid + j] = c[j];
    } else if (tid == 64) {
#pragma clang fp contract(off)
        float thr = 0.f, kappa = 0.f, knee = 1.f, alpha = 0.f, mk = 0.f;
        if (comp_on) {
            thr = denorm(p[cmp0], lo[cmp0], hi[cmp0]);
            const float ratio = denorm(p[cmp0 + 1], lo[cmp0 + 1], hi[cmp0 + 1]);
            const float att = denorm(p[cmp0 + 2], lo[cmp0 + 2], hi[cmp0 + 2]);
            knee = denorm(p[cmp0 + 4], lo[cmp0 + 4], hi[cmp0 + 4]);
            mk = denorm(p[cmp0 + 5], lo[cmp0 + 5], hi[cmp0 + 5]);
            kappa = (1.0f / ratio) - 1.0f;
            const float nat = sr * (att / 1000.0f);
            alpha = (float)exp((double)(-2.1972245773362196f / nat));
        }
        rc[RC_THR] = thr;
        rc[RC_KAPPA] = kappa;
        rc[RC_KNEE] = knee;
        rc[RC_ALPHA] = alpha;
        rc[RC_MAKEUP] = mk;
        rc[RC_ALPHA_C] = (float)pow((double)alpha, (double)kCompChunk);
        rc[RC_LOG2A_C] = alpha > 0.0f ? (float)((double)kCompChunk * log2((double)alpha)) : -1.0e30f;
    } else if (tid == 128) {
#pragma clang fp contract(off)
        float gin = 1.0f;
        const int gi = is_master ? 25 : 0;
        if (gin_on) gin = (float)exp2((double)(denorm(p[gi], lo[gi], hi[gi]) / 20.0f) * 3.321928094887362);
        rc[RC_GIN] = gin;
        coef[30] = gin;
        if (is_master) {
            float gout = 1.0f;
            if (d.flags & MST_USE_OUTPUT_FADER) gout = (float)exp2((double)(denorm(p[24], lo[24], hi[24]) / 20.0f) * 3.321928094887362);
            rc[RC_PANL] = gout;
            rc[RC_PANR] = gout;
        } else {
            const float half_pi = 1.5707963267948966f, two_over_pi = 0.6366197723675814f;
            const float theta = denorm(p[25], lo[25], hi[25]) * half_pi;
            rc[RC_PANL] = sqrtf(((half_pi - theta) * two_over_pi) * (float)cos((double)theta));
            rc[RC_PANR] = sqrtf((theta * two_over_pi) * (float)sin((double)theta));
            rc[RC_SEND] = (d.flags & MST_USE_FX_BUS) ? (float)exp2((double)(denorm(p[26], lo[26], hi[26]) / 20.0f) * 3.321928094887362) : 0.0f;
        }
    } else if (tid == 192 && is_master && a.rc_fx) {
        const float* fp = a.fx_params + (int64_t)mrow * MST_NUM_FX_PARAMS;
        float* o = a.rc_fx + (int64_t)mrow * 24;
        const float mix = check ? 1.0f : denorm(fp[24], d.fx_lo[24], d.fx_hi[24]);
        a.fx_mix[mrow] = mix;
        for (int k = 0; k < 12; ++k) {
            o[k] = denorm(fp[k], d.fx_lo[k], d.fx_hi[k]) * mix;
            o[12 + k] = denorm(fp[12 + k], d.fx_lo[12 + k], d.fx_hi[12 + k]) * 10.0f + 1.0f;
        }
    }
    __syncthreads();
    if (tid < 30) {
        float v = coef[tid];
        if (tid < 3) v *= coef[30];
        rc[RC_SOS + tid] = v;
        coef[tid] = v;
    }
    __syncthreads();
    if (tid < kSections) {
        const float b0 = coef[5 * tid];
        rc[RC_AP + 3 * tid] = coef[5 * tid + 1] / b0;
        rc[RC_AP + 3 * tid + 1] = coef[5 * tid + 2] / b0;
        rc[RC_AP + 3 * tid + 2] = 1.0f / b0;
    }

    double c64[30];
    for (int i = 0; i < 30; ++i) c64[i] = (double)coef[i];
    const int part = blockIdx.y;
    if (part == 0) {
    if (tid < 24) {
        const int which = tid / 12, col = tid % 12;
        double st[12];
        for (int i = 0; i < 12; ++i) st[i] = (i == col) ? 1.0 : 0.0;
        if (which == 0) cascade_step<double>(0.0, c64, st);
        else cascade_adj_step<double>(0.0, c64, st);
        for (int i = 0; i < 12; ++i) mats[which][0][i * 12 + col] = st[i];
    }
    if (tid >= 32 && tid < 34) {
        const int which = tid - 32;
        double st[12];
        for (int i = 0; i < 12; ++i) st[i] = 0.0;
        if (which == 0) cascade_step<double>(1.0, c64, st);
        else cascade_adj_step<double>(1.0, c64, st);
        for (int i = 0; i < 12; ++i) wv[which][0][i] = st[i];
    }
    __syncthreads();

    const int grp = tid / 144, e = tid % 144;
    const bool mat_lane = tid < 288;
    float* powF = (is_master ? a.powF_m + (int64_t)mrow * kPow * 144 : a.powF_t + (int64_t)row * kPow * 144);
    float* powA = (is_master ? a.powA_m + (int64_t)mrow * kPow * 144 : a.powA_t + (int64_t)row * kPow * 144);
    float* pw = grp == 0 ? powF : powA;
    int cur = 0;
    for (int s = 1; s < kEqChunk; s <<= 1) {
        if (a.eq1) {
            for (int item = tid; item < 2 * s * 12; item += 320) {
                const int g2 = item / (s * 12), t = (item / 12) % s, dd = item % 12;
                double acc = 0.0;
#pragma unroll
                for (int q = 0; q < 12; ++q) acc = fma(mats[g2][cur][dd * 12 + q], wv[g2][t][q], acc);
                wv[g2][t + s][dd] = acc;
            }
        }
        if (mat_lane) mat12_mul(mats[grp][cur], mats[grp][cur], mats[grp][cur ^ 1], e);
        __syncthreads();
        cur ^= 1;
    }
    if (mat_lane) pw[0 * 144 + e] = (float)mats[grp][cur][e];
    if (a.eq1) {
        float* wzF = is_master ? a.wzF_m + (int64_t)mrow * kWz : a.wzF_t + (int64_t)row * kWz;
        float* wzA = is_master ? a.wzA_m + (int64_t)mrow * kWz : a.wzA_t + (int64_t)row * kWz;
        for (int item = tid; item < 2 * kWz; item += 320) {
            const int g2 = item / kWz, j = (item % kWz) / 16, dd = item % 16;
            const float v = dd < 12 ? (float)wv[g2][g2 == 0 ? kEqChunk - 1 - j : j][dd] : 0.0f;
            (g2 == 0 ? wzF : wzA)[j * 16 + dd] = v;
        }
    }
    if (a.eq1) {
        float* pw1 = grp == 0 ? (is_master ? a.pow1F_m + (int64_t)mrow * kTri2 : a.pow1F_t + (int64_t)row * kTri2)
                              : (is_master ? a.pow1A_m + (int64_t)mrow * kTri2 : a.pow1A_t + (int64_t)row * kTri2);
        const int ei = e / 12, ec = e % 12, bk = ei >> 1, bj = ec >> 1, sub = (ei & 1) * 2 + (ec & 1);
        constexpr int kPow1Full = 6;
        for (int j = 0; j < kPow1; ++j) {
            if (mat_lane) {
                float* set = pw1 + (j / 6) * (kTri2 / 2);
                const float val = (float)mats[grp][cur][e];
                if (bk == bj) set[(6 * bk + j % 6) * 4 + sub] = val;
                else if (j % 6 == 0 && bj < bk) set[144 + (bk * (bk - 1) / 2 + bj) * 4 + sub] = val;
            }
            if (j % 6 == 0 && tid >= 288 && tid < 300) {
                const int g2 = (tid - 288) / 6, k = (tid - 288) % 6;
                const double* Mm = mats[g2][cur];
                double* o = dblk[j / 6][g2][k];
                o[0] = Mm[(2 * k) * 12 + 2 * k];
                o[1] = Mm[(2 * k) * 12 + 2 * k + 1];
                o[2] = Mm[(2 * k + 1) * 12 + 2 * k];
                o[3] = Mm[(2 * k + 1) * 12 + 2 * k + 1];
            }
            if (j == kPow1Full) break;
            if (mat_lane) mat12_mul(mats[grp][cur], mats[grp][cur], mats[grp][cur ^ 1], e);
            __syncthreads();
            cur ^= 1;
        }
        __syncthreads();
        for (int item = tid; item < 12 * (kPow1 - 1 - kPow1Full); item += 320) {
            const int nj = kPow1 - 1 - kPow1Full, blk = item / nj, jj = item % nj, g2 = blk / 6, k = blk % 6;
            const double* d = dblk[1][g2][k];
            double b0 = d[0], b1 = d[1], b2 = d[2], b3 = d[3];
            for (int sq = 0; sq <= jj; ++sq) {
                const double n0 = fma(b1, b2, b0 * b0), n1 = fma(b1, b3, b0 * b1), n2 = fma(b3, b2, b2 * b0), n3 = fma(b3, b3, b2 * b1);
                b0 = n0; b1 = n1; b2 = n2; b3 = n3;
            }
            float* base = g2 == 0 ? (is_master ? a.pow1F_m + (int64_t)mrow * kTri2 : a.pow1F_t + (int64_t)row * kTri2)
                                  : (is_master ? a.pow1A_m + (int64_t)mrow * kTri2 : a.pow1A_t + (int64_t)row * kTri2);
            const int j = kPow1Full + 1 + jj;
            *reinterpret_cast<float4*>(base + (j / 6) * (kTri2 / 2) + (6 * k + j % 6) * 4) = make_float4((float)b0, (float)b1, (float)b2, (float)b3);
        }
        __syncthreads();
        for (int item = tid; item < 24 * 16; item += 320) {
            const int blk = item >> 4, q = item & 15, set = blk / 12, g2 = (blk / 6) & 1, k = blk % 6;
            const double* d = dblk[set][g2][k];
            double b0 = d[0], b1 = d[1], b2 = d[2], b3 = d[3];
            double r0 = 1.0, r1 = 0.0, r2 = 0.0, r3 = 1.0;
            for (int ebit = q + 1; ebit > 0; ebit >>= 1) {
                if (ebit & 1) {
                    const double n0 = fma(r0, b0, r1 * b2), n1 = fma(r0, b1, r1 * b3), n2 = fma(r2, b0, r3 * b2), n3 = fma(r2, b1, r3 * b3);
                    r0 = n0; r1 = n1; r2 = n2; r3 = n3;
                }
                const double s0_ = fma(b0, b0, b1 * b2), s1_ = fma(b0, b1, b1 * b3), s2_ = fma(b2, b0, b3 * b2), s3_ = fma(b2, b1, b3 * b3);
                b0 = s0_; b1 = s1_; b2 = s2_; b3 = s3_;
            }
            float* base = g2 == 0 ? (is_master ? a.pow1F_m + (int64_t)mrow * kTri2 : a.pow1F_t + (int64_t)row * kTri2)
                                  : (is_master ? a.pow1A_m + (int64_t)mrow * kTri2 : a.pow1A_t + (int64_t)row * kTri2);
            *reinterpret_cast<float4*>(base + set * (kTri2 / 2) + 208 + (16 * k + q) * 4) = make_float4((float)r0, (float)r1, (float)r2, (float)r3);
        }
    } else {
    if (mat_lane) mats[grp][2][e] = (e / 12 == e % 12) ? 1.0 : 0.0;
    __syncthreads();
    for (int k = a.KE; k > 0; k >>= 1) {
        if (k & 1) {
            double tmpv = 0.0;
            if (mat_lane) {
                const int i = e / 12, j = e % 12;
                for (int q = 0; q < 12; ++q) tmpv = fma(mats[grp][2][i * 12 + q], mats[grp][cur][q * 12 + j], tmpv);
            }
            __syncthreads();
            if (mat_lane) mats[grp][2][e] = tmpv;
            __syncthreads();
        }
        if (k > 1) {
            if (mat_lane) mat12_mul(mats[grp][cur], mats[grp][cur], mats[grp][cur ^ 1], e);
            __syncthreads();
            cur ^= 1;
        }
    }
    int src = 2;
    for (int j = 0; j < kScanLevels; ++j) {
        if (mat_lane) pw[(1 + j) * 144 + e] = (float)mats[grp][src][e];
        if (j + 1 < kScanLevels) {
            const int dst = (src == 2) ? 0 : (src == 0 ? 1 : 0);
            if (mat_lane) mat12_mul(mats[grp][src], mats[grp][src], mats[grp][dst], e);
            __syncthreads();
            src = dst;
        }
    }
    }

    }

    if (part == 1 && tid < 12) {
        const int f = tid, k = f >> 1;
        double c1, c2;
        if (f & 1) {
            c1 = c64[5 * k + 1] / c64[5 * k + 0];
            c2 = c64[5 * k + 2] / c64[5 * k + 0];
        } else {
            c1 = c64[5 * k + 3];
            c2 = c64[5 * k + 4];
        }
        double m[4] = {-c1, -c2, 1.0, 0.0}, t[4];
        auto mul = [](const double* x, const double* y, double* o) {
            o[0] = fma(x[0], y[0], x[1] * y[2]);
            o[1] = fma(x[0], y[1], x[1] * y[3]);
            o[2] = fma(x[2], y[0], x[3] * y[2]);
            o[3] = fma(x[2], y[1], x[3] * y[3]);
        };
        for (int s = 1; s < kEqChunk; s <<= 1) {
            mul(m, m, t);
            for (int i = 0; i < 4; ++i) m[i] = t[i];
        }
        float* pp = (is_master ? a.powP_m + ((int64_t)mrow * 12 + f) * kPow * 4 : a.powP_t + ((int64_t)row * 12 + f) * kPow * 4);
        for (int i = 0; i < 4; ++i) pp[i] = (float)m[i];
        double acc[4] = {1, 0, 0, 1}, base[4] = {m[0], m[1], m[2], m[3]};
        for (int k2 = a.KE; k2 > 0; k2 >>= 1) {
            if (k2 & 1) {
                mul(acc, base, t);
                for (int i = 0; i < 4; ++i) acc[i] = t[i];
            }
            mul(base, base, t);
            for (int i = 0; i < 4; ++i) base[i] = t[i];
        }
        for (int j = 0; j < kScanLevels; ++j) {
            for (int i = 0; i < 4; ++i) pp[(1 + j) * 4 + i] = (float)acc[i];
            mul(acc, acc, t);
            for (int i = 0; i < 4; ++i) acc[i] = t[i];
        }
    }
}

__global__ __launch_bounds__(256) void k_prep_bwd(PrepBwdArgs a) {
    __shared__ double dsos[EP_COUNT];
    __shared__ double dcp[CP_COUNT];
    __shared__ double lanesum[64][EP_COUNT + CP_COUNT + 1];
    __shared__ double Jd[kSections][5][3];
    const int row = blockIdx.x, tid = threadIdx.x;
    for (int64_t i = (int64_t)blockIdx.x * 256 + tid; i < a.gran_n; i += (int64_t)gridDim.x * 256) a.gran[i] = 0ull;
    const bool is_master = row >= a.R;
    const int mrow = row - a.R;
    const mst_console_desc& d = a.d;
    const double sr = d.sample_rate;
    const float* p = is_master ? a.master_params + (int64_t)mrow * MST_NUM_MASTER_PARAMS
                               : a.track_params + (int64_t)row * MST_NUM_TRACK_PARAMS;
    const float* lo = is_master ? d.master_lo : d.track_lo;
    const float* hi = is_master ? d.master_hi : d.track_hi;
    const float* rc = is_master ? a.rc_m + (int64_t)mrow * RC_STRIDE : a.rc_t + (int64_t)row * RC_STRIDE;
    float* g = is_master ? a.grad_master_params + (int64_t)mrow * MST_NUM_MASTER_PARAMS
                         : a.grad_track_params + (int64_t)row * MST_NUM_TRACK_PARAMS;
    const int np = is_master ? MST_NUM_MASTER_PARAMS : MST_NUM_TRACK_PARAMS;
    const int eq0 = is_master ? 0 : 1, cmp0 = is_master ? 18 : 19;
    const bool eq_on = is_master ? (d.flags & MST_USE_MASTER_BUS) : (d.flags & MST_USE_TRACK_EQ);
    const bool comp_on = is_master ? (d.flags & MST_USE_MASTER_BUS) : (d.flags & MST_USE_TRACK_COMPRESSOR);
    const bool gin_on = is_master ? (d.flags & MST_USE_MASTER_BUS) : (d.flags & MST_USE_TRACK_INPUT_FADER);
    const bool chain_on = is_master ? (d.flags & MST_USE_MASTER_BUS) : true;

    if (tid < 64) {
        const int nsig = is_master ? 2 : 1;
        const float* ep = is_master ? a.ep_m + ((int64_t)(mrow * 2) * a.nblkEt) * EP_COUNT
                                    : a.ep_t + ((int64_t)row * a.nblkEt) * EP_COUNT;
        const int nE = chain_on ? nsig * a.nblkEt : 0;
        double se[EP_COUNT];
#pragma unroll
        for (int q = 0; q < EP_COUNT; ++q) se[q] = 0.0;
        for (int b = tid; b < nE; b += 64) {
            const float* pb = ep + (int64_t)b * EP_COUNT;
            float2 v[EP_COUNT / 2];
#pragma unroll
            for (int q = 0; q < EP_COUNT / 2; ++q) v[q] = *reinterpret_cast<const float2*>(pb + 2 * q);
#pragma unroll
            for (int q = 0; q < EP_COUNT / 2; ++q) {
                se[2 * q] += (double)v[q].x;
                se[2 * q + 1] += (double)v[q].y;
            }
        }
        const float* cp = is_master ? a.cp_m + ((int64_t)mrow * a.nblkC) * CP_COUNT : a.cp_t + ((int64_t)row * a.nblkC) * CP_COUNT;
        double sc[CP_COUNT];
#pragma unroll
        for (int q = 0; q < CP_COUNT; ++q) sc[q] = 0.0;
        for (int b = tid; b < a.nblkC; b += 64) {
            const float4 v0 = *reinterpret_cast<const float4*>(cp + (int64_t)b * CP_COUNT);
            const float4 v1 = *reinterpret_cast<const float4*>(cp + (int64_t)b * CP_COUNT + 4);
            sc[0] += (double)v0.x; sc[1] += (double)v0.y; sc[2] += (double)v0.z; sc[3] += (double)v0.w;
            sc[4] += (double)v1.x; sc[5] += (double)v1.y; sc[6] += (double)v1.z; sc[7] += (double)v1.w;
        }
#pragma unroll
        for (int q = 0; q < EP_COUNT; ++q) lanesum[tid][q] = se[q];
#pragma unroll
        for (int q = 0; q < CP_COUNT; ++q) lanesum[tid][EP_COUNT + q] = sc[q];
    } else if (tid < 64 + kSections) {
        const int k = tid - 64, i = eq0 + 3 * k;
        if (eq_on) {
            D3 J[5];
            design_section_dual(section_kind(k), (double)denorm(p[i], lo[i], hi[i]), (double)denorm(p[i + 1], lo[i + 1], hi[i + 1]),
                                (double)denorm(p[i + 2], lo[i + 2], hi[i + 2]), sr, J);
            for (int j = 0; j < 5; ++j)
                for (int v = 0; v < 3; ++v) Jd[k][j][v] = J[j].d[v];
        }
    }
    if (tid < np) g[tid] = 0.0f;
    __syncthreads();
    if (tid < EP_COUNT + CP_COUNT) {
        double s = 0.0;
        for (int l = 0; l < 64; ++l) s += lanesum[l][tid];
        if (tid < EP_COUNT) dsos[tid] = s;
        else dcp[tid - EP_COUNT] = s;
    }
    __syncthreads();

    const double gin = rc[RC_GIN];
    if (tid < kSections) {
        if (eq_on) {
            const int k = tid, i = eq0 + 3 * k;
            const double bs0 = (k == 0) ? gin : 1.0;
            for (int v = 0; v < 3; ++v) {
                double acc = 0.0;
                for (int j = 0; j < 5; ++j) acc += dsos[5 * k + j] * Jd[k][j][v] * (j < 3 ? bs0 : 1.0);
                g[i + v] = (float)(acc * (double)(hi[i + v] - lo[i + v]));
            }
        }
    } else if (tid == 64) {
        if (gin_on) {
            double acc = 0.0;
            for (int j = 0; j < 3; ++j) acc += dsos[j] * (double)rc[RC_SOS + j];
            const int gi = is_master ? 25 : 0;
            g[gi] = (float)(acc * (double)kLn10Over20 * (double)(hi[gi] - lo[gi]));
        }
    } else if (tid == 128) {
        if (comp_on) {
            const double ratio = (double)denorm(p[cmp0 + 1], lo[cmp0 + 1], hi[cmp0 + 1]);
            const double att = (double)denorm(p[cmp0 + 2], lo[cmp0 + 2], hi[cmp0 + 2]);
            const double alpha = rc[RC_ALPHA];
            g[cmp0 + 0] = (float)(dcp[CP_THR] * (double)(hi[cmp0] - lo[cmp0]));
            g[cmp0 + 1] = (float)(dcp[CP_KAPPA] * (-1.0 / (ratio * ratio)) * (double)(hi[cmp0 + 1] - lo[cmp0 + 1]));
            g[cmp0 + 2] = (float)(dcp[CP_ALPHA] * alpha * 2.1972245773362196 * 1000.0 / (sr * att * att) *
                                  (double)(hi[cmp0 + 2] - lo[cmp0 + 2]));
            g[cmp0 + 3] = 0.0f;
            g[cmp0 + 4] = (float)(dcp[CP_KNEE] * (double)(hi[cmp0 + 4] - lo[cmp0 + 4]));
            g[cmp0 + 5] = (float)(dcp[CP_MAKEUP] * (double)(hi[cmp0 + 5] - lo[cmp0 + 5]));
        }
    } else if (tid == 192) {
        if (is_master) {
            if (d.flags & MST_USE_OUTPUT_FADER) {
                g[24] = (float)(dcp[CP_PANL] * (double)rc[RC_PANL] * (double)kLn10Over20 * (double)(hi[24] - lo[24]));
            }
        } else {
            const double half_pi = 1.5707963267948966, two_over_pi = 0.6366197723675814;
            const double theta = (double)denorm(p[25], lo[25], hi[25]) * half_pi;
            const double L = rc[RC_PANL], Rr = rc[RC_PANR];
            double dLdth = 0.0, dRdth = 0.0;
            if (L > 0.0) dLdth = (-two_over_pi * cos(theta) - (half_pi - theta) * two_over_pi * sin(theta)) / (2.0 * L);
            if (Rr > 0.0) dRdth = (two_over_pi * sin(theta) + theta * two_over_pi * cos(theta)) / (2.0 * Rr);
            g[25] = (float)((dcp[CP_PANL] * dLdth + dcp[CP_PANR] * dRdth) * half_pi * (double)(hi[25] - lo[25]));
            if (d.flags & MST_USE_FX_BUS)
                g[26] = (float)(dcp[CP_SEND] * (double)rc[RC_SEND] * (double)kLn10Over20 * (double)(hi[26] - lo[26]));
        }
    }
    if (is_master && a.grad_fx_params && tid >= 64 && tid < 64 + MST_NUM_FX_PARAMS) {
        const int k = tid - 64;
        float* gf = a.grad_fx_params + (int64_t)mrow * MST_NUM_FX_PARAMS;
        const double mix = (double)a.fx_mix[mrow];
        if (k == 24) {
            double acc = 0.0;
            if (d.flags & MST_NO_RANGE_CHECK) {
                for (int j = 0; j < 12; ++j) {
                    double aj = 0.0;
                    for (int bk = 0; bk < a.nblkF; ++bk) aj += (double)a.fx_part[((int64_t)mrow * a.nblkF + bk) * 24 + j];
                    acc += aj * (double)denorm(a.fx_params[(int64_t)mrow * MST_NUM_FX_PARAMS + j], d.fx_lo[j], d.fx_hi[j]);
                }
                for (int bk = 0; bk < a.nblkX; ++bk) acc -= (double)a.fx_dry[(int64_t)mrow * a.nblkX + bk];
                acc *= (double)(d.fx_hi[24] - d.fx_lo[24]);
            }
            gf[k] = (float)acc;
        } else {
            double acc = 0.0;
            for (int bk = 0; bk < a.nblkF; ++bk) acc += (double)a.fx_part[((int64_t)mrow * a.nblkF + bk) * 24 + k];
            const double scale = (double)(d.fx_hi[k] - d.fx_lo[k]) * (k >= 12 ? 10.0 : mix);
            gf[k] = (float)(acc * scale);
        }
    }
}

struct BasicConst { float gin, pl, pr; };
__device__ __forceinline__ BasicConst basic_consts(const float* p, const mst_console_desc& d) {
#pragma clang fp contract(off)
    BasicConst k;
    k.gin = 1.0f;
    if (d.flags & MST_USE_TRACK_INPUT_FADER) k.gin = (float)exp2((double)(denorm(p[0], d.track_lo[0], d.track_hi[0]) / 20.0f) * 3.321928094887362);
    const float half_pi = 1.5707963267948966f, two_over_pi = 0.6366197723675814f;
    const float theta = denorm(p[25], d.track_lo[25], d.track_hi[25]) * half_pi;
    k.pl = sqrtf(((half_pi - theta) * two_over_pi) * (float)cos((double)theta));
    k.pr = sqrtf((theta * two_over_pi) * (float)sin((double)theta));
    return k;
}
constexpr int kBasicSpan = 8 * 256;
__global__ __launch_bounds__(256) void k_basic_fwd(BasicArgs a) {
    __shared__ BasicConst kc[kBasicMaxTracks];
    const int b = blockIdx.y, tid = threadIdx.x, T = a.d.n_tracks;
    const float* tp = a.track_params + (int64_t)b * T * MST_NUM_TRACK_PARAMS;
    if (tid < T) kc[tid] = basic_consts(tp + (int64_t)tid * MST_NUM_TRACK_PARAMS, a.d);
    if (blockIdx.x == 0 && !(a.d.flags & MST_NO_RANGE_CHECK)) {
        for (int i = tid; i < T * MST_NUM_TRACK_PARAMS; i += 256) {
            const float v = tp[i];
            if (v < 0.0f || v > 1.0f) atomicMax(a.status, 1000 - (1 + i % MST_NUM_TRACK_PARAMS));
        }
        if (tid < MST_NUM_FX_PARAMS - 1) {
            const float v = a.fx_params[(int64_t)b * MST_NUM_FX_PARAMS + tid];
            if (v < 0.0f || v > 1.0f) atomicMax(a.status, 1000 - (1 + 27 + tid));
        }
        if (tid >= 64 && tid < 64 + MST_NUM_MASTER_PARAMS) {
            const float v = a.master_params[(int64_t)b * MST_NUM_MASTER_PARAMS + tid - 64];
            if (v < 0.0f || v > 1.0f) atomicMax(a.status, 1000 - (1 + 52 + tid - 64));
        }
    }
    __syncthreads();
    const int64_t i0 = (int64_t)blockIdx.x * kBasicSpan + tid * 8, n = a.d.n_samples;
    float4 L[2] = {make_float4(0, 0, 0, 0), make_float4(0, 0, 0, 0)}, R[2] = {L[0], L[0]};
    for (int t = 0; t < T; ++t) {
        const float* row = a.tracks + ((int64_t)b * T + t) * a.d.track_row_stride;
        const BasicConst k = kc[t];
#pragma unroll
        for (int h = 0; h < 2; ++h) {
            const float4 x = load4(row, i0 + 4 * h, n);
            const float4 y = make_float4(k.gin * x.x, k.gin * x.y, k.gin * x.z, k.gin * x.w);
            L[h] = make_float4(fmaf(k.pl, y.x, L[h].x), fmaf(k.pl, y.y, L[h].y), fmaf(k.pl, y.z, L[h].z), fmaf(k.pl, y.w, L[h].w));
            R[h] = make_float4(fmaf(k.pr, y.x, R[h].x), fmaf(k.pr, y.y, R[h].y), fmaf(k.pr, y.z, R[h].z), fmaf(k.pr, y.w, R[h].w));
            if (a.mixed) {
                store4(a.mixed + (((int64_t)b * 2 + 0) * T + t) * n, i0 + 4 * h, n, make_float4(k.pl * y.x, k.pl * y.y, k.pl * y.z, k.pl * y.w));
                store4(a.mixed + (((int64_t)b * 2 + 1) * T + t) * n, i0 + 4 * h, n, make_float4(k.pr * y.x, k.pr * y.y, k.pr * y.z, k.pr * y.w));
            }
        }
    }
#pragma unroll
    for (int h = 0; h < 2; ++h) {
        store4(a.mix + ((int64_t)b * 2 + 0) * n, i0 + 4 * h, n, L[h]);
        store4(a.mix + ((int64_t)b * 2 + 1) * n, i0 + 4 * h, n, R[h]);
    }
}
__global__ __launch_bounds__(256) void k_basic_bwd_part(BasicArgs a) {
    __shared__ BasicConst kc[kBasicMaxTracks];
    __shared__ float red[4][2];
    const int b = blockIdx.y, tid = threadIdx.x, T = a.d.n_tracks;
    if (tid < T) kc[tid] = basic_consts(a.track_params + ((int64_t)b * T + tid) * MST_NUM_TRACK_PARAMS, a.d);
    __syncthreads();
    const int64_t i0 = (int64_t)blockIdx.x * kBasicSpan + tid * 8, n = a.d.n_samples;
    float gl[8], gr[8];
#pragma unroll
    for (int h = 0; h < 2; ++h) {
        const float4 l = load4(a.grad_mix + ((int64_t)b * 2 + 0) * n, i0 + 4 * h, n), r = load4(a.grad_mix + ((int64_t)b * 2 + 1) * n, i0 + 4 * h, n);
        gl[4 * h] = l.x; gl[4 * h + 1] = l.y; gl[4 * h + 2] = l.z; gl[4 * h + 3] = l.w;
        gr[4 * h] = r.x; gr[4 * h + 1] = r.y; gr[4 * h + 2] = r.z; gr[4 * h + 3] = r.w;
    }
    for (int t = 0; t < T; ++t) {
        const float* row = a.tracks + ((int64_t)b * T + t) * a.d.track_row_stride;
        const BasicConst k = kc[t];
        float sl = 0.0f, sr = 0.0f;
#pragma unroll
        for (int h = 0; h < 2; ++h) {
            const float4 x4 = load4(row, i0 + 4 * h, n);
            const float x[4] = {x4.x, x4.y, x4.z, x4.w};
            float ml[4] = {0, 0, 0, 0}, mr[4] = {0, 0, 0, 0};
            if (a.grad_mixed) {
                const float4 u = load4(a.grad_mixed + (((int64_t)b * 2 + 0) * T + t) * n, i0 + 4 * h, n);
                const float4 v = load4(a.grad_mixed + (((int64_t)b * 2 + 1) * T + t) * n, i0 + 4 * h, n);
                ml[0] = u.x; ml[1] = u.y; ml[2] = u.z; ml[3] = u.w;
                mr[0] = v.x; mr[1] = v.y; mr[2] = v.z; mr[3] = v.w;
            }
            float gx[4];
#pragma unroll
            for (int e = 0; e < 4; ++e) {
                const float y = k.gin * x[e], cl = gl[4 * h + e] + ml[e], cr = gr[4 * h + e] + mr[e];
                sl = fmaf(cl, y, sl);
                sr = fmaf(cr, y, sr);
                gx[e] = k.gin * fmaf(k.pr, cr, k.pl * cl);
            }
            if (a.grad_tracks) store4(a.grad_tracks + ((int64_t)b * T + t) * n, i0 + 4 * h, n, make_float4(gx[0], gx[1], gx[2], gx[3]));
        }
        sl = wave_sum(sl);
        sr = wave_sum(sr);
        if ((tid & 63) == 0) { red[tid >> 6][0] = sl; red[tid >> 6][1] = sr; }
        __syncthreads();
        if (tid < 2) a.part[(((int64_t)b * gridDim.x + blockIdx.x) * T + t) * 2 + tid] = (red[0][tid] + red[1][tid]) + (red[2][tid] + red[3][tid]);
        __syncthreads();
    }
}
__global__ void k_basic_bwd_final(BasicArgs a, int nblk) {
    const int r = blockIdx.x * blockDim.x + threadIdx.x, T = a.d.n_tracks;
    if (r >= a.d.bs * T) return;
    const int b = r / T, t = r % T;
    double sl = 0.0, sr = 0.0;
    for (int k = 0; k < nblk; ++k) {
        sl += (double)a.part[(((int64_t)b * nblk + k) * T + t) * 2];
        sr += (double)a.part[(((int64_t)b * nblk + k) * T + t) * 2 + 1];
    }
    const float* p = a.track_params + (int64_t)r * MST_NUM_TRACK_PARAMS;
    const BasicConst k = basic_consts(p, a.d);
    float* g = a.grad_track_params + (int64_t)r * MST_NUM_TRACK_PARAMS;
    for (int i = 0; i < MST_NUM_TRACK_PARAMS; ++i) g[i] = 0.0f;
    const float* lo = a.d.track_lo;
    const float* hi = a.d.track_hi;
    if (a.d.flags & MST_USE_TRACK_INPUT_FADER)
        g[0] = (float)(((double)k.pl * sl + (double)k.pr * sr) * (double)kLn10Over20 * (double)(hi[0] - lo[0]));
    const double half_pi = 1.5707963267948966, two_over_pi = 0.6366197723675814;
    const double theta = (double)denorm(p[25], lo[25], hi[25]) * half_pi, L = k.pl, Rr = k.pr;
    double dLdth = 0.0, dRdth = 0.0;
    if (L > 0.0) dLdth = (-two_over_pi * cos(theta) - (half_pi - theta) * two_over_pi * sin(theta)) / (2.0 * L);
    if (Rr > 0.0) dRdth = (two_over_pi * sin(theta) + theta * two_over_pi * cos(theta)) / (2.0 * Rr);
    g[25] = (float)((sl * dLdth + sr * dRdth) * half_pi * (double)(hi[25] - lo[25]));
    if (t == 0 && a.grad_master_params)
        for (int i = 0; i < MST_NUM_MASTER_PARAMS; ++i) a.grad_master_params[(int64_t)b * MST_NUM_MASTER_PARAMS + i] = 0.0f;
}
void launch_basic_forward(const BasicArgs& a, hipStream_t stream) {
    const int nblk = (int)((a.d.n_samples + kBasicSpan - 1) / kBasicSpan);
    hipLaunchKernelGGL(k_basic_fwd, dim3(nblk, a.d.bs), dim3(256), 0, stream, a);
}
void launch_basic_backward(const BasicArgs& a, hipStream_t stream) {
    const int nblk = (int)((a.d.n_samples + kBasicSpan - 1) / kBasicSpan), rows = a.d.bs * a.d.n_tracks;
    hipLaunchKernelGGL(k_basic_bwd_part, dim3(nblk, a.d.bs), dim3(256), 0, stream, a);
    hipLaunchKernelGGL(k_basic_bwd_final, dim3((rows + 63) / 64), dim3(64), 0, stream, a, nblk);
}

void launch_prep(const PrepArgs& a, hipStream_t stream) {
#ifndef MST_PREP_PREFETCH_SEGS
#define MST_PREP_PREFETCH_SEGS 12
#endif
    const int segs = (a.pf_src && MST_PREP_PREFETCH_SEGS > 0) ? MST_PREP_PREFETCH_SEGS : 0;
    hipLaunchKernelGGL(k_prep, dim3(a.R + a.bs, 2 + segs), dim3(320), 0, stream, a);
}
void launch_prep_bwd(const PrepBwdArgs& a, hipStream_t stream) {
    hipLaunchKernelGGL(k_prep_bwd, dim3(a.R + a.bs), dim3(256), 0, stream, a);
}

}
```

Measured before the change: 18280.

## Compute fused all-pole bank chunk states with MFMA against precomputed impulse-response matrix

Replaces the per-sample serial all-pole recursion (six sections × two filters, run per sample inside the forward EQ loop) with a matrix product. The prep kernel now builds each row's truncated impulse responses into a 64×32 weight matrix. The cascade kernel multiplies each tile slab by it using 16x16x4 f32 MFMA, then transposes the accumulators through LDS to write the zero-state outputs. This takes a long dependent FMA chain off the hot loop. In exchange it adds a workspace buffer, extra LDS traffic and syncs, and a prep-kernel stage whose correctness depends on matching the exact lane layout.

After: 17910. 2.0% lower.

```diff
diff --git a/diff-mst_amd/csrc/mst_common.h b/diff-mst_amd/csrc/mst_common.h
--- a/diff-mst_amd/csrc/mst_common.h
+++ b/diff-mst_amd/csrc/mst_common.h
@@ -24,6 +24,7 @@
 constexpr int kTri2 = 2 * 592;
 constexpr int kFxDhChunks = 4;
 constexpr int kWz = kEqChunk * 16;
+constexpr int kWp = kEqChunk * 32;
 constexpr int kMaxTiles1 = 64;
 
 constexpr int RC_SOS = 0;
@@ -299,6 +300,7 @@
     int64_t pow1F_t, pow1F_m, pow1A_t, pow1A_m;
     int64_t aggF_t, aggF_m, aggA_t, aggA_m;
     int64_t wzF_t, wzF_m, wzA_t, wzA_m;
+    int64_t wp_t, wp_m;
     int64_t gran_f, gran_b;
     int64_t gran_nf, gran_nb;
     int64_t eqg_f, eqg_b;
@@ -397,6 +399,8 @@
     L.wzF_m = L.wzF_t + R * kWz;
     L.wzA_t = take((R + B) * kWz);
     L.wzA_m = L.wzA_t + R * kWz;
+    L.wp_t = take((R + B) * kWp);
+    L.wp_m = L.wp_t + R * kWp;
     L.eqg_nf = (R + 2 * B) * kMaxTiles1 * kStates;
     L.eqg_nb = 2 * B * kMaxTiles1 * kStates;
     L.gran_nf = 2 * B * L.nblkC + 2 * L.eqg_nf;
diff --git a/diff-mst_amd/csrc/mst_console.hip b/diff-mst_amd/csrc/mst_console.hip
--- a/diff-mst_amd/csrc/mst_console.hip
+++ b/diff-mst_amd/csrc/mst_console.hip
@@ -100,7 +100,7 @@
 
     PrepArgs pa{track_params, fx_bus_params, master_bus_params, ws + L.rc_t, ws + L.rc_m,
                 ws + L.powF_t, ws + L.powF_m, ws + L.powA_t, ws + L.powA_m, ws + L.powP_t, ws + L.powP_m,
-                ws + L.pow1F_t, ws + L.pow1F_m, ws + L.pow1A_t, ws + L.pow1A_m, ws + L.wzF_t, ws + L.wzF_m, ws + L.wzA_t, ws + L.wzA_m, fx_on ? ws + L.fx_rc : nullptr, fx_on ? ws + L.fx_mix : nullptr, status, L.R, L.bs, L.KE,
+                ws + L.pow1F_t, ws + L.pow1F_m, ws + L.pow1A_t, ws + L.pow1A_m, ws + L.wzF_t, ws + L.wzF_m, ws + L.wzA_t, ws + L.wzA_m, ws + L.wp_t, ws + L.wp_m, fx_on ? ws + L.fx_rc : nullptr, fx_on ? ws + L.fx_mix : nullptr, status, L.R, L.bs, L.KE,
                 L.eq1, *d, (gran_t*)(ws + L.gran_f), L.gran_nf + L.gran_nb, nullptr, 0, 0};
 #ifndef MST_PREP_RIDER_MAX_BYTES
 #define MST_PREP_RIDER_MAX_BYTES (128ll << 20)
@@ -136,9 +136,9 @@
     if (!L.eq1) launch_scan12(false, ws + L.zE_t, ws + L.sE_t, ws + L.powF_t, L.R, L.ncE, L.ncE_pad, L.KE, L.R, stream);
     if (t_comp)
         launch_cascade_run_gc(tracks, d->track_row_stride, ws + L.u_t, Ns, ws + L.rc_t, L.R, sE_t, L.ncE_pad, n, L.R,
-                              ws + L.zS_t, L.nblkC, stream, p1F_t, L.ntE, ws + L.aggF_t, zP_t, zsin_t ? &zi_t : nullptr);
+                              ws + L.zS_t, L.nblkC, stream, p1F_t, L.ntE, ws + L.aggF_t, zP_t, zsin_t ? &zi_t : nullptr, ws + L.wp_t);
     else
-        launch_cascade(EQ_FWD, true, tracks, d->track_row_stride, ws + L.u_t, Ns, ws + L.rc_t, L.R, sE_t, nullptr, L.ncE_pad, n, L.R, stream, p1F_t, L.ntE, ws + L.aggF_t, zP_t);
+        launch_cascade(EQ_FWD, true, tracks, d->track_row_stride, ws + L.u_t, Ns, ws + L.rc_t, L.R, sE_t, nullptr, L.ncE_pad, n, L.R, stream, p1F_t, L.ntE, ws + L.aggF_t, zP_t, ws + L.wp_t);
     const bool bus_is_mix = !m_on && !o_on;
     float* busp = bus_is_mix ? mix : ws + L.bus;
     const int64_t bus_stride = bus_is_mix ? n : Ns;
@@ -157,10 +157,10 @@
         else launch_cascade(EQ_FWD, false, ws + L.bus, Ns, nullptr, 0, ws + L.rc_m, 0, nullptr, ws + L.zE_m, L.ncE_pad, n, 2 * L.bs, stream, p1F_m, L.ntE, ws + L.aggF_m);
         if (!L.eq1) launch_scan12(false, ws + L.zE_m, ws + L.sE_m, ws + L.powF_m, 0, L.ncE, L.ncE_pad, L.KE, 2 * L.bs, stream);
         if (apscan_m)
-            launch_master_run_apscan(ws + L.bus, Ns, ws + L.v_m, Ns, ws + L.rc_m, sE_m, L.ncE_pad, n, 2 * L.bs, stream, p1F_m, L.ntE, ws + L.aggF_m, zP_m,
+            launch_master_run_apscan(ws + L.bus, Ns, ws + L.v_m, Ns, ws + L.rc_m, sE_m, L.ncE_pad, n, 2 * L.bs, stream, p1F_m, L.ntE, ws + L.aggF_m, zP_m, ws + L.wp_m,
                                      ws + L.zP_t, ws + L.sP_t, ws + L.powP_t, L.R * 12, L.ncE, L.apscan_sh, EQ_FWD, zsin_m ? &zi_m : nullptr);
         else
-            launch_cascade(EQ_FWD, true, ws + L.bus, Ns, ws + L.v_m, Ns, ws + L.rc_m, 0, sE_m, nullptr, L.ncE_pad, n, 2 * L.bs, stream, p1F_m, L.ntE, ws + L.aggF_m, zP_m);
+            launch_cascade(EQ_FWD, true, ws + L.bus, Ns, ws + L.v_m, Ns, ws + L.rc_m, 0, sE_m, nullptr, L.ncE_pad, n, 2 * L.bs, stream, p1F_m, L.ntE, ws + L.aggF_m, zP_m, ws + L.wp_m);
         MasterApplyArgs ma{ws + L.v_m, Ns, ws + L.rc_m, ws + L.zS_m, save ? ws + L.gs_m : nullptr, mix, n,
                            L.ncC_pad, d->master_lookahead, 1, n, aligned, (gran_t*)(ws + L.gran_f), (int64_t)L.bs * L.nblkC, status};
         launch_apply_master(ma, L.bs, stream);
@@ -289,7 +289,7 @@
         if (!L.eq1) launch_scan12(true, ws + L.zA_m, ws + L.sA_m, ws + L.powA_m, 0, L.ncE, L.ncE_pad, L.KE, 2 * L.bs, stream);
         if (master_cg_later)
             launch_master_run_apscan(ws + L.du_m, Ns, ws + L.dbus, Ns, ws + L.rc_m, ws + L.zA_m, L.ncE_pad, n, 2 * L.bs, stream, p1A_m, L.ntE, ws + L.aggA_m,
-                                     nullptr, ws + L.zP_m, ws + L.sP_m, ws + L.powP_m, 2 * L.bs * 12, L.ncE, L.apscan_sh, EQ_ADJ, zsin_a ? &zi_a : nullptr);
+                                     nullptr, nullptr, ws + L.zP_m, ws + L.sP_m, ws + L.powP_m, 2 * L.bs * 12, L.ncE, L.apscan_sh, EQ_ADJ, zsin_a ? &zi_a : nullptr);
         else
             launch_cascade(EQ_ADJ, true, ws + L.du_m, Ns, ws + L.dbus, Ns, ws + L.rc_m, 0, L.eq1 ? ws + L.zA_m : ws + L.sA_m, nullptr, L.ncE_pad, n,
                            2 * L.bs, stream, p1A_m, L.ntE, ws + L.aggA_m);
diff --git a/diff-mst_amd/csrc/mst_eq.hip b/diff-mst_amd/csrc/mst_eq.hip
--- a/diff-mst_amd/csrc/mst_eq.hip
+++ b/diff-mst_amd/csrc/mst_eq.hip
@@ -103,7 +103,7 @@
                                                  int nc_pad, int64_t n, float* __restrict__ zs_comp,
                                                  int nblk_comp, const float* __restrict__ pw1, int ntiles,
                                                  float* __restrict__ agg, float* __restrict__ tile, float* __restrict__ zp,
-                                                 const int sig, const int bx, const ZsIn zi = ZsIn{}) {
+                                                 const float* __restrict__ wp, const int sig, const int bx, const ZsIn zi = ZsIn{}) {
     static_assert(!ZSIN || (MODE_RUN && SCAN1), "the in-launch zero-state pass belongs to the SCAN1 run");
     const int tid = threadIdx.x;
     const int64_t tile_base = (int64_t)bx * kEqWG * kEqChunk;
@@ -178,14 +178,12 @@
     CompK ck{};
     float zacc = 0.0f;
     if (FUSE_GC) ck = load_comp(rc + (int64_t)filter_row(sig, split) * RC_STRIDE);
-    f2 nk1[kSections], nk2[kSections], w1[kSections], w2[kSections];
+    const int li = tid & 15, g = tid >> 4;
+    f32x4_t ap[4][2];
+    const float* apw = FUSE_AP ? wp + (int64_t)filter_row(sig, split) * kWp + (4 * g) * 32 + li : nullptr;
     if (FUSE_AP) {
 #pragma unroll
-        for (int s = 0; s < kSections; ++s) {
-            nk1[s] = f2{-c[5 * s + 3], -coef[RC_AP - RC_SOS + 3 * s]};
-            nk2[s] = f2{-c[5 * s + 4], -coef[RC_AP - RC_SOS + 3 * s + 1]};
-            w1[s] = w2[s] = f2{0.0f, 0.0f};
-        }
+        for (int m = 0; m < 4; ++m) ap[m][0] = ap[m][1] = f32x4_t{0.f, 0.f, 0.f, 0.f};
     }
 
 #ifndef MST_EQ_PACKED
@@ -224,18 +222,6 @@
                 v.z = step_fwd(v.z);
                 v.w = step_fwd(v.w);
                 if (MODE_RUN) *reinterpret_cast<float4*>(&mine[i4]) = v;
-                if (FUSE_AP) {
-                    const float ys[4] = {v.x, v.y, v.z, v.w};
-#pragma unroll
-                    for (int t = 0; t < 4; ++t) {
-#pragma unroll
-                        for (int s = 0; s < kSections; ++s) {
-                            const f2 wn = f2_fma(nk2[s], w2[s], f2_fma(nk1[s], w1[s], f2{ys[t], ys[t]}));
-                            w2[s] = w1[s];
-                            w1[s] = wn;
-                        }
-                    }
-                }
                 if (FUSE_GC) {
                     float dd;
                     zacc = fmaf(ck.alpha, zacc, ck.oma * gain_computer(v.x, ck, dd));
@@ -258,6 +244,25 @@
         wave_lds_sync();
         if (MODE_RUN) {
             slab_store<FAST>(tile, outrow, tile_base, j, n, tid);
+            if (FUSE_AP) {
+                __builtin_amdgcn_sched_barrier(0);
+                float apb[4][2];
+#pragma unroll
+                for (int e = 0; e < 4; ++e) {
+                    apb[e][0] = apw[(kSlab * j + e) * 32];
+                    apb[e][1] = apw[(kSlab * j + e) * 32 + 16];
+                }
+#pragma unroll
+                for (int m = 0; m < 4; ++m) {
+                    const float4 y4 = *reinterpret_cast<const float4*>(&tile[(16 * m + li) * kLdw + 4 * g]);
+                    const float y[4] = {y4.x, y4.y, y4.z, y4.w};
+#pragma unroll
+                    for (int e = 0; e < 4; ++e) {
+                        ap[m][0] = __builtin_amdgcn_mfma_f32_16x16x4f32(y[e], apb[e][0], ap[m][0], 0, 0, 0);
+                        ap[m][1] = __builtin_amdgcn_mfma_f32_16x16x4f32(y[e], apb[e][1], ap[m][1], 0, 0, 0);
+                    }
+                }
+            }
             wave_lds_sync();
         }
     }
@@ -282,13 +287,20 @@
         }
     }
     if (FUSE_AP) {
-#pragma unroll
-        for (int s = 0; s < kSections; ++s) {
-            const int64_t base = ((int64_t)sig * 24 + 4 * s) * nc_pad + chunk;
-            zp[base] = w1[s].x;
-            zp[base + nc_pad] = w2[s].x;
-            zp[base + 2 * (int64_t)nc_pad] = w1[s].y;
-            zp[base + 3 * (int64_t)nc_pad] = w2[s].y;
+        constexpr int kPitch = 17;
+        static_assert(kEqWG * kPitch <= kEqWG * kLdw, "the transposition fits the slab image");
+#pragma unroll
+        for (int nb = 0; nb < 2; ++nb) {
+            if (nb == 0 || li < 8) {
+#pragma unroll
+                for (int m = 0; m < 4; ++m)
+#pragma unroll
+                    for (int r = 0; r < 4; ++r) tile[(16 * m + 4 * g + r) * kPitch + li] = ap[m][nb][r];
+            }
+            wave_lds_sync();
+#pragma unroll
+            for (int q = 0; q < (nb == 0 ? 16 : 8); ++q) zp[((int64_t)sig * 24 + 16 * nb + q) * nc_pad + chunk] = tile[tid * kPitch + q];
+            wave_lds_sync();
         }
     }
     if (FUSE_GC) {
@@ -317,14 +329,15 @@
                                                  const float* __restrict__ s0, float* __restrict__ z,
                                                  int nc_pad, int64_t n, float* __restrict__ zs_comp = nullptr,
                                                  int nblk_comp = 0, const float* __restrict__ pw1 = nullptr, int ntiles = 0,
-                                                 float* __restrict__ agg = nullptr, float* __restrict__ zp = nullptr) {
+                                                 float* __restrict__ agg = nullptr, float* __restrict__ zp = nullptr,
+                                                 const float* __restrict__ wp = nullptr) {
     static_assert(!FUSE_AP || (MODE_RUN && DIR == EQ_FWD), "the all-pole bank rides on the forward run only");
     __shared__ __attribute__((aligned(16))) float tile[kEqWG * kLdw > kTriFloats ? kEqWG * kLdw : kTriFloats];
     const int64_t tile_base = (int64_t)blockIdx.x * kTile;
     const bool fast = tile_fast(in + (int64_t)blockIdx.y * in_stride, tile_base, n) &&
                       (!MODE_RUN || !((uintptr_t)(out + (int64_t)blockIdx.y * out_stride) & 15));
-    if (fast) cascade_body<DIR, MODE_RUN, FUSE_GC, SCAN1, true, FUSE_AP>(in, in_stride, out, out_stride, rc, split, s0, z, nc_pad, n, zs_comp, nblk_comp, pw1, ntiles, agg, tile, zp, blockIdx.y, blockIdx.x);
-    else cascade_body<DIR, MODE_RUN, FUSE_GC, SCAN1, false, FUSE_AP>(in, in_stride, out, out_stride, rc, split, s0, z, nc_pad, n, zs_comp, nblk_comp, pw1, ntiles, agg, tile, zp, blockIdx.y, blockIdx.x);
+    if (fast) cascade_body<DIR, MODE_RUN, FUSE_GC, SCAN1, true, FUSE_AP>(in, in_stride, out, out_stride, rc, split, s0, z, nc_pad, n, zs_comp, nblk_comp, pw1, ntiles, agg, tile, zp, wp, blockIdx.y, blockIdx.x);
+    else cascade_body<DIR, MODE_RUN, FUSE_GC, SCAN1, false, FUSE_AP>(in, in_stride, out, out_stride, rc, split, s0, z, nc_pad, n, zs_comp, nblk_comp, pw1, ntiles, agg, tile, zp, wp, blockIdx.y, blockIdx.x);
 }
 
 template <int DIR, bool FUSE_GC, bool FUSE_AP>
@@ -332,15 +345,15 @@
                                                  float* __restrict__ out, int64_t out_stride,
                                                  const float* __restrict__ rc, int split, int nc_pad, int64_t n,
                                                  float* __restrict__ zs_comp, int nblk_comp, const float* __restrict__ pw1, int ntiles,
-                                                 float* __restrict__ zp, ZsIn zi) {
+                                                 float* __restrict__ zp, const float* __restrict__ wp, ZsIn zi) {
     __shared__ __attribute__((aligned(16))) float tile[kEqWG * kLdw > kTriFloats ? kEqWG * kLdw : kTriFloats];
     int sig, step;
     row_block_xcd(sig, step);
     const int bx = DIR == EQ_FWD ? step : ntiles - 1 - step;
     const int64_t tile_base = (int64_t)bx * kTile;
     const bool fast = tile_fast(in + (int64_t)sig * in_stride, tile_base, n) && !((uintptr_t)(out + (int64_t)sig * out_stride) & 15);
-    if (fast) cascade_body<DIR, true, FUSE_GC, true, true, FUSE_AP, true>(in, in_stride, out, out_stride, rc, split, nullptr, nullptr, nc_pad, n, zs_comp, nblk_comp, pw1, ntiles, nullptr, tile, zp, sig, bx, zi);
-    else cascade_body<DIR, true, FUSE_GC, true, false, FUSE_AP, true>(in, in_stride, out, out_stride, rc, split, nullptr, nullptr, nc_pad, n, zs_comp, nblk_comp, pw1, ntiles, nullptr, tile, zp, sig, bx, zi);
+    if (fast) cascade_body<DIR, true, FUSE_GC, true, true, FUSE_AP, true>(in, in_stride, out, out_stride, rc, split, nullptr, nullptr, nc_pad, n, zs_comp, nblk_comp, pw1, ntiles, nullptr, tile, zp, wp, sig, bx, zi);
+    else cascade_body<DIR, true, FUSE_GC, true, false, FUSE_AP, true>(in, in_stride, out, out_stride, rc, split, nullptr, nullptr, nc_pad, n, zs_comp, nblk_comp, pw1, ntiles, nullptr, tile, zp, wp, sig, bx, zi);
 }
 
 template <int DIR>
@@ -461,7 +474,8 @@
 __global__ __launch_bounds__(kEqWG) void k_master_run_apscan(const float* __restrict__ in, int64_t in_stride, float* __restrict__ out,
                                                            int64_t out_stride, const float* __restrict__ rc, const float* __restrict__ s0,
                                                            int nc_pad, int64_t n, const float* __restrict__ pw1, int ntiles,
-                                                           float* __restrict__ agg, float* __restrict__ zp, int nsig, ApScanArgs sc, ZsIn zi) {
+                                                           float* __restrict__ agg, float* __restrict__ zp, const float* __restrict__ wp, int nsig,
+                                                           ApScanArgs sc, ZsIn zi) {
     __shared__ __attribute__((aligned(16))) float tile[2 * kEqWG * kLdw > kTriFloats ? 2 * kEqWG * kLdw : kTriFloats];
     if ((int)blockIdx.y >= nsig) {
         const int job = ((int)blockIdx.y - nsig) * gridDim.x + blockIdx.x;
@@ -483,17 +497,17 @@
     const int64_t tile_base = (int64_t)bx * kTile;
     const bool fast = tile_fast(in + (int64_t)sig * in_stride, tile_base, n) && !((uintptr_t)(out + (int64_t)sig * out_stride) & 15);
     constexpr bool AP = DIR == EQ_FWD;
-    if (fast) cascade_body<DIR, true, false, true, true, AP, ZSIN>(in, in_stride, out, out_stride, rc, 0, s0, nullptr, nc_pad, n, nullptr, 0, pw1, ntiles, agg, tile, zp, sig, bx, zi);
-    else cascade_body<DIR, true, false, true, false, AP, ZSIN>(in, in_stride, out, out_stride, rc, 0, s0, nullptr, nc_pad, n, nullptr, 0, pw1, ntiles, agg, tile, zp, sig, bx, zi);
+    if (fast) cascade_body<DIR, true, false, true, true, AP, ZSIN>(in, in_stride, out, out_stride, rc, 0, s0, nullptr, nc_pad, n, nullptr, 0, pw1, ntiles, agg, tile, zp, wp, sig, bx, zi);
+    else cascade_body<DIR, true, false, true, false, AP, ZSIN>(in, in_stride, out, out_stride, rc, 0, s0, nullptr, nc_pad, n, nullptr, 0, pw1, ntiles, agg, tile, zp, wp, sig, bx, zi);
 }
 void launch_master_run_apscan(const float* in, int64_t in_stride, float* out, int64_t out_stride, const float* rc, const float* s0, int nc_pad,
-                              int64_t n, int nsig, hipStream_t stream, const float* pw1, int ntiles, float* agg, float* zp,
+                              int64_t n, int nsig, hipStream_t stream, const float* pw1, int ntiles, float* agg, float* zp, const float* wp,
                               const float* sc_z, float* sc_s0, const float* sc_tab, int sc_jobs, int sc_nc, int sc_sh, int dir, const ZsIn* zi) {
     const ApScanArgs sc{sc_z, sc_s0, sc_tab, sc_jobs, sc_nc, nc_pad, sc_sh, dir == EQ_ADJ ? 1 : 0};
     const dim3 grid(ntiles, nsig + (sc_jobs + ntiles - 1) / ntiles), block(kEqWG);
     const ZsIn z0 = zi ? *zi : ZsIn{};
 #define MST_LAUNCH_MRA(D, Z) \
-    hipLaunchKernelGGL(HIP_KERNEL_NAME(k_master_run_apscan<D, Z>), grid, block, 0, stream, in, in_stride, out, out_stride, rc, s0, nc_pad, n, pw1, ntiles, agg, zp, nsig, sc, z0)
+    hipLaunchKernelGGL(HIP_KERNEL_NAME(k_master_run_apscan<D, Z>), grid, block, 0, stream, in, in_stride, out, out_stride, rc, s0, nc_pad, n, pw1, ntiles, agg, zp, wp, nsig, sc, z0)
     if (dir == EQ_FWD) {
         if (z0.wz) MST_LAUNCH_MRA(EQ_FWD, true);
         else MST_LAUNCH_MRA(EQ_FWD, false);
@@ -506,21 +520,21 @@
 
 void launch_cascade(int dir, bool run, const float* in, int64_t in_stride, float* out, int64_t out_stride, const float* rc,
                     int split, const float* s0, float* z, int nc_pad, int64_t n, int nsig, hipStream_t stream, const float* pw1,
-                    int ntiles, float* agg, float* zp) {
+                    int ntiles, float* agg, float* zp, const float* wp) {
     const dim3 grid(pw1 ? ntiles : nc_pad / kEqWG, nsig), block(kEqWG);
     float* const nozs = nullptr;
     if (zp && dir == EQ_FWD && run) {
         if (pw1)
             hipLaunchKernelGGL(HIP_KERNEL_NAME(k_cascade<EQ_FWD, true, false, true, true>), grid, block, 0, stream, in, in_stride, out,
-                               out_stride, rc, split, s0, z, nc_pad, n, nozs, 0, pw1, ntiles, agg, zp);
+                               out_stride, rc, split, s0, z, nc_pad, n, nozs, 0, pw1, ntiles, agg, zp, wp);
         else
             hipLaunchKernelGGL(HIP_KERNEL_NAME(k_cascade<EQ_FWD, true, false, false, true>), grid, block, 0, stream, in, in_stride, out,
-                               out_stride, rc, split, s0, z, nc_pad, n, nozs, 0, pw1, ntiles, agg, zp);
+                               out_stride, rc, split, s0, z, nc_pad, n, nozs, 0, pw1, ntiles, agg, zp, wp);
         return;
     }
 #define MST_LAUNCH_CASCADE(D, R, S) \
     hipLaunchKernelGGL(HIP_KERNEL_NAME(k_cascade<D, R, false, S>), grid, block, 0, stream, in, in_stride, out, out_stride, rc, \
-                       split, s0, z, nc_pad, n, nozs, 0, pw1, ntiles, agg, nozs)
+                       split, s0, z, nc_pad, n, nozs, 0, pw1, ntiles, agg, nozs, wp)
     if (pw1) {
         if (dir == EQ_FWD && !run) MST_LAUNCH_CASCADE(EQ_FWD, false, true);
         else if (dir == EQ_FWD) MST_LAUNCH_CASCADE(EQ_FWD, true, true);
@@ -537,29 +551,29 @@
 
 void launch_cascade_run_gc(const float* in, int64_t in_stride, float* out, int64_t out_stride, const float* rc, int split,
                            const float* s0, int nc_pad, int64_t n, int nsig, float* zs_comp, int nblk_comp, hipStream_t stream,
-                           const float* pw1, int ntiles, float* agg, float* zp, const ZsIn* zi) {
+                           const float* pw1, int ntiles, float* agg, float* zp, const ZsIn* zi, const float* wp) {
     static_assert(kWG * kCompChunk % kEqChunk == 0 && kEqWG % (kWG * kCompChunk / kEqChunk) == 0, "a compressor block must be a power-of-two group of EQ lanes");
     const dim3 grid(pw1 ? ntiles : nc_pad / kEqWG, nsig), block(kEqWG);
     if (zi && zi->wz && pw1) {
-        if (zp) hipLaunchKernelGGL(HIP_KERNEL_NAME(k_cascade_zsin<EQ_FWD, true, true>), grid, block, 0, stream, in, in_stride, out, out_stride, rc, split, nc_pad, n, zs_comp, nblk_comp, pw1, ntiles, zp, *zi);
-        else hipLaunchKernelGGL(HIP_KERNEL_NAME(k_cascade_zsin<EQ_FWD, true, false>), grid, block, 0, stream, in, in_stride, out, out_stride, rc, split, nc_pad, n, zs_comp, nblk_comp, pw1, ntiles, zp, *zi);
+        if (zp) hipLaunchKernelGGL(HIP_KERNEL_NAME(k_cascade_zsin<EQ_FWD, true, true>), grid, block, 0, stream, in, in_stride, out, out_stride, rc, split, nc_pad, n, zs_comp, nblk_comp, pw1, ntiles, zp, wp, *zi);
+        else hipLaunchKernelGGL(HIP_KERNEL_NAME(k_cascade_zsin<EQ_FWD, true, false>), grid, block, 0, stream, in, in_stride, out, out_stride, rc, split, nc_pad, n, zs_comp, nblk_comp, pw1, ntiles, zp, wp, *zi);
         return;
     }
     if (zp) {
         if (pw1)
             hipLaunchKernelGGL(HIP_KERNEL_NAME(k_cascade<EQ_FWD, true, true, true, true>), grid, block, 0, stream, in, in_stride, out, out_stride,
-                               rc, split, s0, (float*)nullptr, nc_pad, n, zs_comp, nblk_comp, pw1, ntiles, agg, zp);
+                               rc, split, s0, (float*)nullptr, nc_pad, n, zs_comp, nblk_comp, pw1, ntiles, agg, zp, wp);
         else
             hipLaunchKernelGGL(HIP_KERNEL_NAME(k_cascade<EQ_FWD, true, true, false, true>), grid, block, 0, stream, in, in_stride, out, out_stride,
-                               rc, split, s0, (float*)nullptr, nc_pad, n, zs_comp, nblk_comp, pw1, ntiles, agg, zp);
+                               rc, split, s0, (float*)nullptr, nc_pad, n, zs_comp, nblk_comp, pw1, ntiles, agg, zp, wp);
         return;
     }
     if (pw1)
         hipLaunchKernelGGL(HIP_KERNEL_NAME(k_cascade<EQ_FWD, true, true, true>), grid, block, 0, stream, in, in_stride, out, out_stride,
-                           rc, split, s0, (float*)nullptr, nc_pad, n, zs_comp, nblk_comp, pw1, ntiles, agg, (float*)nullptr);
+                           rc, split, s0, (float*)nullptr, nc_pad, n, zs_comp, nblk_comp, pw1, ntiles, agg, (float*)nullptr, wp);
     else
         hipLaunchKernelGGL(HIP_KERNEL_NAME(k_cascade<EQ_FWD, true, true, false>), grid, block, 0, stream, in, in_stride, out, out_stride,
-                           rc, split, s0, (float*)nullptr, nc_pad, n, zs_comp, nblk_comp, pw1, ntiles, agg, (float*)nullptr);
-}
-
-}
+                           rc, split, s0, (float*)nullptr, nc_pad, n, zs_comp, nblk_comp, pw1, ntiles, agg, (float*)nullptr, wp);
+}
+
+}
diff --git a/diff-mst_amd/csrc/mst_kernels.h b/diff-mst_amd/csrc/mst_kernels.h
--- a/diff-mst_amd/csrc/mst_kernels.h
+++ b/diff-mst_amd/csrc/mst_kernels.h
@@ -18,6 +18,7 @@
     float* pow1A_t; float* pow1A_m;
     float* wzF_t; float* wzF_m;
     float* wzA_t; float* wzA_m;
+    float* wp_t; float* wp_m;
     float* rc_fx;
     float* fx_mix;
     int32_t* status;
@@ -86,14 +87,15 @@
 };
 void launch_cascade(int dir, bool run, const float* in, int64_t in_stride, float* out, int64_t out_stride, const float* rc,
                     int split, const float* s0, float* z, int nc_pad, int64_t n, int nsig, hipStream_t stream,
-                    const float* pw1 = nullptr, int ntiles = 0, float* agg = nullptr, float* zp = nullptr);
+                    const float* pw1 = nullptr, int ntiles = 0, float* agg = nullptr, float* zp = nullptr, const float* wp = nullptr);
 void launch_cascade_run_gc(const float* in, int64_t in_stride, float* out, int64_t out_stride, const float* rc, int split,
                            const float* s0, int nc_pad, int64_t n, int nsig, float* zs_comp, int nblk_comp, hipStream_t stream,
-                           const float* pw1 = nullptr, int ntiles = 0, float* agg = nullptr, float* zp = nullptr, const ZsIn* zi = nullptr);
+                           const float* pw1 = nullptr, int ntiles = 0, float* agg = nullptr, float* zp = nullptr, const ZsIn* zi = nullptr,
+                           const float* wp = nullptr);
 void launch_eq_zs_mfma(int dir, const float* in, int64_t in_stride, const float* wz, int split, float* z, int nc_pad, int64_t n, int nsig,
                        hipStream_t stream, const float* pw1, int ntiles, float* agg);
 void launch_master_run_apscan(const float* in, int64_t in_stride, float* out, int64_t out_stride, const float* rc, const float* s0, int nc_pad,
-                              int64_t n, int nsig, hipStream_t stream, const float* pw1, int ntiles, float* agg, float* zp,
+                              int64_t n, int nsig, hipStream_t stream, const float* pw1, int ntiles, float* agg, float* zp, const float* wp,
                               const float* sc_z, float* sc_s0, const float* sc_tab, int sc_jobs, int sc_nc, int sc_sh, int dir = EQ_FWD,
                               const ZsIn* zi = nullptr);
 
diff --git a/diff-mst_amd/csrc/mst_params.hip b/diff-mst_amd/csrc/mst_params.hip
--- a/diff-mst_amd/csrc/mst_params.hip
+++ b/diff-mst_amd/csrc/mst_params.hip
@@ -392,8 +392,26 @@
 
     }
 
-    if (part == 1 && tid < 12) {
+    if (part == 1) {
+    float* wps = reinterpret_cast<float*>(&wv[0][0][0]);
+    static_assert(sizeof(wv) >= kWp * sizeof(float), "the all-pole map is staged in wv");
+    for (int i = tid; i < kEqChunk * 8; i += 320) wps[(i >> 3) * 32 + 24 + (i & 7)] = 0.0f;
+    if (tid < 12) {
         const int f = tid, k = f >> 1;
+        {
+            const double n1 = -(double)((f & 1) ? coef[5 * k + 1] / coef[5 * k] : coef[5 * k + 3]);
+            const double n2 = -(double)((f & 1) ? coef[5 * k + 2] / coef[5 * k] : coef[5 * k + 4]);
+            const int col = 4 * k + 2 * (f & 1);
+            double h1 = 0.0, h2 = 0.0;
+            wps[(kEqChunk - 1) * 32 + col + 1] = 0.0f;
+            for (int nn = 0; nn < kEqChunk; ++nn) {
+                const double h = fma(n2, h2, fma(n1, h1, nn == 0 ? 1.0 : 0.0));
+                wps[(kEqChunk - 1 - nn) * 32 + col] = (float)h;
+                if (nn + 1 < kEqChunk) wps[(kEqChunk - 2 - nn) * 32 + col + 1] = (float)h;
+                h2 = h1;
+                h1 = h;
+            }
+        }
         double c1, c2;
         if (f & 1) {
             c1 = c64[5 * k + 1] / c64[5 * k + 0];
@@ -429,6 +447,10 @@
             mul(acc, acc, t);
             for (int i = 0; i < 4; ++i) acc[i] = t[i];
         }
+    }
+    __syncthreads();
+    float2* wpo = reinterpret_cast<float2*>(is_master ? a.wp_m + (int64_t)mrow * kWp : a.wp_t + (int64_t)row * kWp);
+    for (int i = tid; i < kWp / 2; i += 320) wpo[i] = reinterpret_cast<const float2*>(wps)[i];
     }
 }
 
```
